# kscalelabs/kbot-joystick

Measured on NVIDIA B200. Metric: env-steps/sec (obs + LSTM actor/critic + torque + terminations + rewards + GAE), higher is better.
Workload: dtype f32 (tcgen05 2xFP16-split GEMMs, fp32 accumulate)

## Files before the change

### kbot-joystick_b200/csrc/kbs_api.cu

```cuda
#include <math.h>
#include <stdio.h>
#include <stdlib.h>
#include <string.h>

#include <new>

#include "kbs_common.cuh"

namespace {

inline int64_t round_up4(int64_t n) { return (n + 3) / 4 * 4; }

int check_ld(int64_t ld, int64_t n) {
  if (n <= 0) return KBS_E_SHAPE;
  if (ld < round_up4(n)) return KBS_E_SHAPE;
  if (ld % 4) return KBS_E_ALIGN;
  return KBS_OK;
}

#define REQ(p)            \
  do {                    \
    if (!(p)) return KBS_E_NULL; \
  } while (0)
#define AL(p)                                     \
  do {                                            \
    if ((p) && !kbs_aligned16(p)) return KBS_E_ALIGN; \
  } while (0)

int check_state(const kbs_state_view* s, int64_t n, bool need_priv) {
  REQ(s);
  REQ(s->qpos); REQ(s->qvel);
  int rc = check_ld(s->ld, n);
  if (rc) return rc;
  AL(s->qpos); AL(s->qvel); AL(s->sensordata); AL(s->xpos); AL(s->xquat); AL(s->cinert); AL(s->cvel);
  AL(s->actuator_force); AL(s->com_distance); AL(s->time);
  if (need_priv) { REQ(s->sensordata); REQ(s->xpos); REQ(s->xquat); }
  return KBS_OK;
}

kbs_state_view state_at(const kbs_state_view& s, int64_t t) {
  kbs_state_view o = s;
  const int64_t ld = s.ld;
  if (s.qpos) o.qpos = s.qpos + t * KBS_NQ * ld;
  if (s.qvel) o.qvel = s.qvel + t * KBS_NV * ld;
  if (s.sensordata) o.sensordata = s.sensordata + t * KBS_NSENSORDATA * ld;
  if (s.xpos) o.xpos = s.xpos + t * 3 * KBS_NBODY * ld;
  if (s.xquat) o.xquat = s.xquat + t * 4 * KBS_NBODY * ld;
  if (s.cinert) o.cinert = s.cinert + t * 10 * KBS_NBODY * ld;
  if (s.cvel) o.cvel = s.cvel + t * 6 * KBS_NBODY * ld;
  if (s.actuator_force) o.actuator_force = s.actuator_force + t * KBS_NUM_JOINTS * ld;
  if (s.com_distance) o.com_distance = s.com_distance + t * ld;
  if (s.time) o.time = s.time + t * ld;
  return o;
}

kbs_noise_view noise_at(const kbs_noise_view& z, int64_t t, int64_t ld) {
  kbs_noise_view o = z;
  if (z.eps_jpos) o.eps_jpos = z.eps_jpos + t * 20 * ld;
  if (z.eps_jvel) o.eps_jvel = z.eps_jvel + t * 20 * ld;
  if (z.eps_gyro) o.eps_gyro = z.eps_gyro + t * 3 * ld;
  if (z.eps_pg) o.eps_pg = z.eps_pg + t * 3 * ld;
  return o;
}

size_t trunk_scratch_floats(const kbs_handle* h, int64_t n) {
  return h->p.gemm_path != KBS_GEMM_SIMT_FP32 ? kbs_tc_scratch_floats(h, n) : kbs_simt_scratch_floats(h, n);
}

int trunk(kbs_handle* h, int net, const float* obs, int64_t ld, float* carry, const uint8_t* done, float* out_rm,
          int64_t n, cudaStream_t st) {
  if (h->p.gemm_path == KBS_GEMM_SIMT_FP32) return kbs_simt_trunk(h, net, obs, ld, carry, done, out_rm, n, st);
  const size_t H = size_t(h->p.hidden_size);
  float* ws = h->scratch;
  float* x_rm = ws + kbs_tc_scratch_floats(h, n) - 2 * size_t(n) * H - 256;
  float* hbuf = x_rm + size_t(n) * H;
  int rc;
  if ((rc = kbs_simt_in_proj(h, net, obs, ld, x_rm, n, st))) return rc;
  if ((rc = kbs_tc_lstm_stack(h, net, x_rm, carry, done, hbuf, ws, n, false, st))) return rc;
  return kbs_simt_out_proj(h, net, hbuf, out_rm, n, st);
}

constexpr int kOutLd = 64;

int rollout_fused_tc(kbs_handle* h, const kbs_rollout_io* io, int64_t n, cudaStream_t st) {
  const int64_t ld = io->state.ld, T = io->T;
  const bool critic = io->value != nullptr;
  int chunks_cfg = 1;
  {
    const char* e = getenv("KBS_ROLLOUT_CHUNKS");
    chunks_cfg = e ? atoi(e) : 1;
    if (chunks_cfg < 1 || chunks_cfg > kKbsMaxChunks) chunks_cfg = 1;
  }
  const int64_t CT = (T + chunks_cfg - 1) / chunks_cfg;
  const size_t sbf = size_t(kbs_tc_sb_floats(h, n));
  const size_t ws_f = kbs_tc_rollout_ws_floats(h, n);
  const size_t lag_f = io->pg_carry ? size_t(T) * 3 * ld : 0;
  const size_t aobs_f = io->actor_obs ? 0 : size_t(T) * KBS_ACTOR_OBS * ld;
  const size_t cobs_f = critic ? size_t(CT) * KBS_CRITIC_OBS * ld : 0;
  const size_t xsb_f = size_t(T) * sbf;
  const size_t osb_a_f = size_t(kbs_tc_obs_sb_floats(h, KBS_NET_ACTOR, n, CT));
  const size_t osb_c_f = critic ? size_t(kbs_tc_obs_sb_floats(h, KBS_NET_CRITIC, n, CT)) : 0;
  int rc = kbs_scratch_reserve(h, ws_f + lag_f + aobs_f + cobs_f + xsb_f * (critic ? 2 : 1) + osb_a_f + osb_c_f + 64);
  if (rc) return rc;
  float* ws = h->scratch;
  float* lagged = io->pg_carry ? ws + ws_f : nullptr;
  float* aobs = io->actor_obs ? io->actor_obs : ws + ws_f + lag_f;
  float* cobs = critic ? ws + ws_f + lag_f + aobs_f : nullptr;
  float* xsb_a = ws + ws_f + lag_f + aobs_f + cobs_f;
  float* xsb_c = critic ? xsb_a + xsb_f : nullptr;
  float* osb_a = xsb_a + xsb_f * (critic ? 2 : 1);
  float* osb_c = critic ? osb_a + osb_a_f : nullptr;

  if ((rc = kbs_launch_terminate(h, io->state, io->term_codes, io->done, io->success, nullptr, n, st, T))) return rc;
  if (lagged) {
    if ((rc = kbs_launch_phase_a_scans(h, io->command, io->u_switch, io->cmd_mode, io->cmd_u6, io->cmd_u_arms, io->done,
                                       io->state.sensordata, io->episode.pg_lag, io->pg_carry, lagged, T, ld, n, st)))
      return rc;
  } else if ((rc = kbs_launch_command_scan(h, io->command, io->u_switch, io->cmd_mode, io->cmd_u6, io->cmd_u_arms, io->done,
                                           T, ld, n, st))) {
    return rc;
  }
  if ((rc = kbs_side_stream_init(h))) return rc;
  const bool overlap = chunks_cfg > 1;
  cudaStream_t aux = overlap ? h->aux_stream : st;
  if (overlap) {
    KBS_CUDA_TRY(cudaEventRecord(h->ev_pre, st));
    KBS_CUDA_TRY(cudaStreamWaitEvent(aux, h->ev_pre, 0));
  }
  KbsTcRolloutArgs r{};
  r.x_sb_all[0] = xsb_a; r.x_sb_all[1] = xsb_c;
  int n_chunks = 0;
  for (int64_t t0 = 0; t0 < T; t0 += CT, ++n_chunks) {
    const int64_t tc = (T - t0 < CT) ? T - t0 : CT;
    const kbs_state_view s = state_at(io->state, t0);
    const kbs_noise_view nz = noise_at(io->noise, t0, ld);
    float* aobs_c = aobs + t0 * KBS_ACTOR_OBS * ld;
    if ((rc = kbs_launch_observations(h, s, &nz, &io->episode, io->command + t0 * KBS_NUM_COMMANDS * ld, nullptr, nullptr,
                                      nullptr, aobs_c, cobs, n, aux, tc, lagged ? lagged + t0 * 3 * ld : nullptr,
                                      true)))
      return rc;
    const float* obs_soa[2] = {aobs_c, cobs};
    float* obs_sb[2] = {osb_a, osb_c};
    float* xsb[2] = {xsb_a + size_t(t0) * sbf, critic ? xsb_c + size_t(t0) * sbf : nullptr};
    if ((rc = kbs_tc_input_proj_all(h, critic ? 2 : 1, obs_soa, obs_sb, xsb, ld, n, tc, aux,
                                    critic ? s.cinert : nullptr, critic ? s.cvel : nullptr, chunks_cfg == 1 ? &r : nullptr)))
      return rc;
    if (overlap) KBS_CUDA_TRY(cudaEventRecord(h->ev_chunk[n_chunks], aux));
  }

  r.chunk_len = overlap ? CT : 0; r.chunk_events = h->ev_chunk;
  r.n = n; r.ld = ld; r.T = T; r.with_critic = critic;
  r.carry[0] = io->actor_carry; r.carry[1] = io->critic_carry;
  r.done = io->done; r.actor_obs = aobs; r.lpf = io->lpf; r.eps_action = io->eps_action;
  r.qpos = io->state.qpos; r.qvel = io->state.qvel; r.ep = io->episode;
  r.action = io->action; r.log_prob = io->log_prob; r.ctrl = io->ctrl; r.value = io->value;
  r.ws = ws;
  return kbs_tc_rollout_recurrent(h, r, st);
}

}

int kbs_side_stream_init(kbs_handle* h) {
  if (h->side_stream) return 0;
  KBS_CUDA_TRY(cudaStreamCreateWithFlags(&h->side_stream, cudaStreamNonBlocking));
  KBS_CUDA_TRY(cudaStreamCreateWithFlags(&h->aux_stream, cudaStreamNonBlocking));
  KBS_CUDA_TRY(cudaEventCreateWithFlags(&h->ev_pre, cudaEventDisableTiming));
  for (int i = 0; i < kKbsMaxChunks; ++i) KBS_CUDA_TRY(cudaEventCreateWithFlags(&h->ev_chunk[i], cudaEventDisableTiming));
  for (int i = 0; i < 2; ++i) {
    KBS_CUDA_TRY(cudaEventCreateWithFlags(&h->ev_lstm[i], cudaEventDisableTiming));
    KBS_CUDA_TRY(cudaEventCreateWithFlags(&h->ev_head[i], cudaEventDisableTiming));
  }
  return 0;
}

int kbs_status_init(kbs_handle* h) {
  if (h->persist_status) return KBS_OK;
  KBS_CUDA_TRY(cudaMalloc(&h->persist_status, 256));
  KBS_CUDA_TRY(cudaMemset(h->persist_status, 0, 256));
  KBS_CUDA_TRY(cudaHostAlloc(&h->status_host, 64, cudaHostAllocDefault));
  *h->status_host = 0u;
  return KBS_OK;
}

int kbs_status_publish(kbs_handle* h, cudaStream_t st) {
  if (!h->persist_status) return KBS_OK;
  KBS_CUDA_TRY(cudaMemcpyAsync(h->status_host, h->persist_status, 4, cudaMemcpyDeviceToHost, st));
  return KBS_OK;
}

int kbs_enter(kbs_handle* h) {
  int dev = -1;
  KBS_CUDA_TRY(cudaGetDevice(&dev));
  if (dev != h->device) return KBS_E_STATE;
  if (h->status_host && *reinterpret_cast<volatile unsigned int*>(h->status_host) != 0u) return KBS_E_DEVICE;
  return KBS_OK;
}

int kbs_scratch_reserve(kbs_handle* h, size_t floats) {
  if (floats <= h->scratch_floats) return KBS_OK;
  if (h->scratch_locked) return KBS_E_STATE;
  if (h->scratch) { KBS_CUDA_TRY(cudaFree(h->scratch)); h->scratch = nullptr; h->scratch_floats = 0; }
  const size_t want = floats + floats / 8 + 1024;
  KBS_CUDA_TRY(cudaMalloc(&h->scratch, want * sizeof(float)));
  h->scratch_floats = want;
  return KBS_OK;
}

extern "C" {

int kbs_version(void) { return KBS_VERSION; }

const char* kbs_error_string(int code) {
  switch (code) {
    case KBS_OK: return "ok";
    case KBS_E_NULL: return "required pointer is NULL";
    case KBS_E_SHAPE: return "unsupported shape (n_envs / ld / T / hidden_size)";
    case KBS_E_ALIGN: return "pointer not 16-byte aligned or ld % 4 != 0";
    case KBS_E_STATE: return "handle not ready (weights not packed, or datapath unavailable)";
    case KBS_E_PARAM: return "bad scalar parameter";
    case KBS_E_DEVICE: return "device health word set (dependency-wait timeout or FP16-split operand out of range): kbs_device_status";
    default: return code > 0 ? cudaGetErrorString((cudaError_t)code) : "unknown kbs error";
  }
}

int kbs_default_params(kbs_params* p) {
  REQ(p);
  memset(p, 0, sizeof(*p));
  p->hidden_size = 256; p->depth = 2; p->gemm_path = KBS_GEMM_SIMT_FP32; p->normalize_advantages = 0;
  p->ctrl_dt = 0.02f; p->min_std = 0.01f; p->max_std = 1.0f; p->var_scale = 0.5f;
  {
    const double w = 2.0 * M_PI * 10.0, dt = 0.02;
    p->lpf_alpha = (float)(w * dt / (1.0 + w * dt));
  }
  p->gamma = 0.94f; p->lam = 0.94f; p->adv_eps = 1e-6f;
  p->jpos_noise_mag = (float)(3.0 * M_PI / 180.0); p->jvel_noise_mag = (float)(15.0 * M_PI / 180.0);
  p->gyro_noise_std = (float)(10.0 * M_PI / 180.0); p->pg_noise_std = (float)(3.0 * M_PI / 180.0);
// ... 337 lines not shown
  return kbs_launch_torque(h, action, *s, ep, ctrl_out, n, (cudaStream_t)stream);
}

int kbs_torque_substeps(kbs_handle* h, const float* action, float* prev_action, const float* u_drop, const float* latency,
                        const float* q_sub, const float* qd_sub, const kbs_episode_view* ep, float* ctrl_out, int32_t n_substeps,
                        float sub_dt, float drop_prob, int64_t ld, int64_t n, void* stream) {
  REQ(h); REQ(action); REQ(prev_action); REQ(u_drop); REQ(latency); REQ(q_sub); REQ(qd_sub); REQ(ctrl_out);
  if (n_substeps <= 0 || n_substeps > 64) return KBS_E_SHAPE;
  int rc = check_ld(ld, n);
  if (rc) return rc;
  AL(action); AL(prev_action); AL(u_drop); AL(latency); AL(q_sub); AL(qd_sub); AL(ctrl_out);
  return kbs_launch_torque_substeps(h, action, prev_action, u_drop, latency, q_sub, qd_sub, ep, ctrl_out, n_substeps, sub_dt,
                                    drop_prob, ld, n, (cudaStream_t)stream);
}

int kbs_terminate(kbs_handle* h, const kbs_state_view* s, int32_t* codes, uint8_t* done, uint8_t* success, float* pre,
                  int64_t n, void* stream) {
  REQ(h);
  int rc = check_state(s, n, false);
  if (rc) return rc;
  REQ(s->xpos); REQ(s->time);
  AL(codes); AL(pre);
  if ((reinterpret_cast<uintptr_t>(done) & 3u) || (reinterpret_cast<uintptr_t>(success) & 3u)) return KBS_E_ALIGN;
  return kbs_launch_terminate(h, *s, codes, done, success, pre, n, (cudaStream_t)stream);
}

int kbs_rewards(kbs_handle* h, const kbs_traj_view* traj, const kbs_reward_carry* carry, float* total,
                float* components, int64_t n, void* stream) {
  REQ(h); REQ(traj); REQ(carry); REQ(total);
  if (traj->T <= 0 || traj->T > 65535) return KBS_E_SHAPE;
  int rc = check_state(&traj->state, n, true);
  if (rc) return rc;
  REQ(traj->state.com_distance); REQ(traj->command); REQ(traj->ctrl); REQ(traj->done);
  REQ(carry->t_single); REQ(carry->airtime); REQ(carry->prev_contact);
  AL(traj->command); AL(traj->ctrl); AL(total); AL(components);
  if (reinterpret_cast<uintptr_t>(traj->done) & 3u) return KBS_E_ALIGN;
  return kbs_launch_rewards(h, *traj, *carry, total, components, n, (cudaStream_t)stream);
}

int kbs_gae(kbs_handle* h, const float* values, const float* rewards, const uint8_t* done, const uint8_t* success,
            float* advantages, float* value_targets, int64_t T, int64_t ld, int64_t n, void* stream) {
  REQ(h); REQ(values); REQ(rewards); REQ(done); REQ(success); REQ(advantages); REQ(value_targets);
  if (T <= 0) return KBS_E_SHAPE;
  if (n <= 0 || ld < n) return KBS_E_SHAPE;
  return kbs_launch_gae(h, values, rewards, done, success, advantages, value_targets, T, ld, n, (cudaStream_t)stream);
}

int kbs_policy_step(kbs_handle* h, const float* joint_angles, const float* joint_vel, const float* projected_gravity,
                    const float* gyro, const float* command, const float* carry_in, float* carry_out,
                    float* action_out, int64_t n, void* stream) {
  REQ(h); REQ(joint_angles); REQ(joint_vel); REQ(projected_gravity); REQ(gyro); REQ(command); REQ(carry_in);
  REQ(carry_out); REQ(action_out);
  if (n <= 0) return KBS_E_SHAPE;
  { const int rc0 = kbs_enter(h); if (rc0) return rc0; }
  cudaStream_t st = (cudaStream_t)stream;
  const int H = h->p.hidden_size, d2 = 2 * h->p.depth;
  const int64_t ld = round_up4(n);
  {
    const char* legacy_env = getenv("KBS_TC_PER_STEP");
    if (h->p.gemm_path != KBS_GEMM_SIMT_FP32 && !(legacy_env && atoi(legacy_env)) && d2 <= 8 &&
        kbs_tc_persistent_available(h, n, 1, 1)) {
      const int carry_w = d2 * H + 20;
      const size_t ws_f = kbs_tc_rollout_ws_floats(h, n);
      const size_t xsb_f = size_t(kbs_tc_sb_floats(h, n));
      const size_t osb_f = size_t(kbs_tc_obs_sb_floats(h, KBS_NET_ACTOR, n, 1));
      int rc = kbs_scratch_reserve(h, ws_f + xsb_f + osb_f + size_t(KBS_ACTOR_OBS + 20 + 20) * ld + 64);
      if (rc) return rc;
      float* ws = h->scratch;
      float* xsb = ws + ws_f;
      float* osb = xsb + xsb_f;
      float* obs = osb + osb_f;
      float* lpf = obs + size_t(KBS_ACTOR_OBS) * ld;
      float* act = lpf + 20 * ld;
      if ((rc = kbs_launch_policy_pack(h, joint_angles, joint_vel, projected_gravity, gyro, command, carry_in, obs, nullptr,
                                       lpf, ld, n, st)))
        return rc;
      const float* obs_soa[2] = {obs, nullptr};
      float* obs_sb[2] = {osb, nullptr};
      float* x_all[2] = {xsb, nullptr};
      KbsTcRolloutArgs r{};
      if ((rc = kbs_tc_input_proj_all(h, 1, obs_soa, obs_sb, x_all, ld, n, 1, st, nullptr, nullptr, &r))) return rc;
      r.n = n; r.ld = ld; r.T = 1; r.with_critic = false;
      r.carry[0] = const_cast<float*>(carry_in); r.carry_out[0] = carry_out; r.carry_ld = carry_w;
      r.actor_obs = obs; r.lpf = lpf; r.action = act;
      r.ws = ws;
      if ((rc = kbs_tc_rollout_recurrent(h, r, st))) return rc;
      return kbs_launch_policy_unpack(h, nullptr, lpf, act, carry_out, action_out, ld, n, st);
    }
  }
  const size_t ts = trunk_scratch_floats(h, n);
  const size_t need = ts + size_t(n) * kOutLd + size_t(KBS_ACTOR_OBS + 20 + 20) * ld + size_t(d2) * n * H + 64;
  int rc = kbs_scratch_reserve(h, need);
  if (rc) return rc;
  float* out_rm = h->scratch + ts;
  float* obs = out_rm + size_t(n) * kOutLd;
  float* lpf = obs + size_t(KBS_ACTOR_OBS) * ld;
  float* mean = lpf + 20 * ld;
  float* carry = mean + 20 * ld;
  if ((rc = kbs_launch_policy_pack(h, joint_angles, joint_vel, projected_gravity, gyro, command, carry_in, obs, carry,
                                   lpf, ld, n, st)))
    return rc;
  if ((rc = trunk(h, KBS_NET_ACTOR, obs, ld, carry, nullptr, out_rm, n, st))) return rc;
  kbs_actor_out o{};
  o.mean = mean;
  if ((rc = kbs_launch_actor_head(h, out_rm, kOutLd, obs, ld, lpf, nullptr, nullptr, nullptr, o, n, st))) return rc;
  return kbs_launch_policy_unpack(h, carry, lpf, mean, carry_out, action_out, ld, n, st);
}

static int ppo_variables_pass(kbs_handle* h, const kbs_ppo_io* io, int64_t n, cudaStream_t st, size_t base, size_t* end_out,
                              bool dry) {
  int rc;
  const bool critic = io->critic_obs != nullptr;
  const int64_t ld = io->ld, T = io->T;
  if (h->p.gemm_path == KBS_GEMM_SIMT_FP32) {
    const size_t ts = trunk_scratch_floats(h, n);
    if (end_out) *end_out = ts + size_t(n) * kOutLd;
    if (dry) return KBS_OK;
    float* out_rm = h->scratch + ts;
    for (int64_t t = 0; t < T; ++t) {
      const uint8_t* done_t = io->done + t * ld;
      if ((rc = trunk(h, KBS_NET_ACTOR, io->actor_obs + t * KBS_ACTOR_OBS * ld, ld, io->actor_carry, done_t, out_rm, n, st)))
        return rc;
      kbs_actor_out o{};
      o.log_prob = io->log_probs ? io->log_probs + t * ld : nullptr;
      o.entropy = io->entropy ? io->entropy + t * ld : nullptr;
      o.std = io->action_std ? io->action_std + t * KBS_NUM_JOINTS * ld : nullptr;
      o.mean = io->mean ? io->mean + t * KBS_NUM_JOINTS * ld : nullptr;
      if ((rc = kbs_launch_actor_head(h, out_rm, kOutLd, io->actor_obs + t * KBS_ACTOR_OBS * ld, ld, io->lpf, nullptr,
                                      io->action + t * KBS_NUM_JOINTS * ld, done_t, o, n, st)))
        return rc;
      if (critic) {
        if ((rc = trunk(h, KBS_NET_CRITIC, io->critic_obs + t * KBS_CRITIC_OBS * ld, ld, io->critic_carry, done_t, out_rm,
                        n, st)))
          return rc;
        if ((rc = kbs_launch_critic_head(h, out_rm, kOutLd, io->values + t * ld, n, st))) return rc;
      }
    }
    return KBS_OK;
  }
  const size_t sbf = size_t(kbs_tc_sb_floats(h, n));
  const size_t ws_f = kbs_tc_rollout_ws_floats(h, n), xsb_f = size_t(T) * sbf;
  const size_t osb_a_f = size_t(kbs_tc_obs_sb_floats(h, KBS_NET_ACTOR, n, T));
  const size_t osb_c_f = critic ? size_t(kbs_tc_obs_sb_floats(h, KBS_NET_CRITIC, n, T)) : 0;
  if (end_out) *end_out = base + ws_f + xsb_f * (critic ? 2 : 1) + osb_a_f + osb_c_f + 64;
  if (dry) return KBS_OK;
  float* ws = h->scratch + base;
  float* xsb_a = ws + ws_f;
  float* xsb_c = critic ? xsb_a + xsb_f : nullptr;
  float* osb_a = xsb_a + xsb_f * (critic ? 2 : 1);
  float* osb_c = critic ? osb_a + osb_a_f : nullptr;
  KbsTcRolloutArgs r{};
  {
    const float* obs_soa[2] = {io->actor_obs, io->critic_obs};
    float* obs_sb[2] = {osb_a, osb_c};
    float* xsb[2] = {xsb_a, xsb_c};
    if ((rc = kbs_tc_input_proj_all(h, critic ? 2 : 1, obs_soa, obs_sb, xsb, ld, n, T, st, nullptr, nullptr, &r))) return rc;
  }
  r.n = n; r.ld = ld; r.T = T; r.with_critic = critic;
  r.carry[0] = io->actor_carry; r.carry[1] = io->critic_carry;
  r.done = io->done; r.actor_obs = io->actor_obs; r.lpf = io->lpf;
  r.action_in = io->action; r.log_prob = io->log_probs; r.entropy = io->entropy; r.action_std = io->action_std;
  r.mean = io->mean;
  r.value = io->values;
  r.ws = ws;
  return kbs_tc_rollout_recurrent(h, r, st);
}

int kbs_ppo_variables(kbs_handle* h, const kbs_ppo_io* io, int64_t n, void* stream) {
  REQ(h); REQ(io);
  REQ(io->actor_obs); REQ(io->action); REQ(io->done); REQ(io->actor_carry); REQ(io->lpf); REQ(io->log_probs);
  REQ(io->entropy);
  if (io->T <= 0) return KBS_E_SHAPE;
  int rc = check_ld(io->ld, n);
  if (rc) return rc;
  if ((rc = kbs_enter(h))) return rc;
  const bool critic = io->critic_obs != nullptr;
  if (critic) { REQ(io->critic_carry); REQ(io->values); }
  AL(io->actor_obs); AL(io->critic_obs); AL(io->action); AL(io->lpf); AL(io->log_probs); AL(io->values); AL(io->entropy);
  AL(io->action_std); AL(io->mean);
  const bool mirror = io->actor_obs_mirror != nullptr;
  if (mirror) {
    REQ(io->actor_mirror_carry); REQ(io->lpf_mirror); REQ(io->action_mirror_loss);
    if (io->critic_obs_mirror) { REQ(io->critic_mirror_carry); REQ(io->value_mirror_loss); if (!critic) return KBS_E_NULL; }
    AL(io->actor_obs_mirror); AL(io->critic_obs_mirror); AL(io->lpf_mirror); AL(io->action_mirror_loss); AL(io->value_mirror_loss);
  }
  cudaStream_t st = (cudaStream_t)stream;
  const int64_t ld = io->ld, T = io->T;
  const bool tc = h->p.gemm_path != KBS_GEMM_SIMT_FP32;
  if (tc && io->mean && !kbs_tc_persistent_available(h, n, T, critic ? 2 : 1)) return KBS_E_SHAPE;
  const size_t mir_f = mirror ? (2 * size_t(T) * KBS_NUM_JOINTS * ld + 3 * size_t(T) * ld + 255) / 256 * 256 : 0;
  size_t pass_end = 0;
  if ((rc = ppo_variables_pass(h, io, n, st, tc ? mir_f : 0, &pass_end, true))) return rc;
  if ((rc = kbs_scratch_reserve(h, pass_end + (tc ? 0 : mir_f) + 64))) return rc;
  float* mir = mirror ? (tc ? h->scratch : h->scratch + pass_end) : nullptr;
  kbs_ppo_io a = *io;
  if (mirror && !a.mean) a.mean = mir;
  if ((rc = ppo_variables_pass(h, &a, n, st, tc ? mir_f : 0, nullptr, false))) return rc;
  if (!mirror) return KBS_OK;
  float* mean_m = mir + size_t(T) * KBS_NUM_JOINTS * ld;
  float* value_m = mean_m + size_t(T) * KBS_NUM_JOINTS * ld;
  float* lp_m = value_m + size_t(T) * ld;
  float* ent_m = lp_m + size_t(T) * ld;
  kbs_ppo_io m = *io;
  m.actor_obs = io->actor_obs_mirror; m.critic_obs = io->critic_obs_mirror;
  m.actor_carry = io->actor_mirror_carry; m.critic_carry = io->critic_mirror_carry; m.lpf = io->lpf_mirror;
  m.log_probs = lp_m; m.entropy = ent_m; m.values = io->critic_obs_mirror ? value_m : nullptr; m.action_std = nullptr;
  m.mean = mean_m;
  if ((rc = ppo_variables_pass(h, &m, n, st, tc ? mir_f : 0, nullptr, false))) return rc;
  return kbs_launch_mirror_loss(h, a.mean, mean_m, io->values, value_m, io->action_mirror_loss,
                                io->critic_obs_mirror ? io->value_mirror_loss : nullptr, io->actor_mirror_loss_scale,
                                io->critic_mirror_loss_scale, T, ld, n, st);
}

int kbs_generate_rollout_noise(kbs_handle* h, uint64_t seed, int64_t step0, const kbs_noise_view* noise, float* eps_action,
                               float* u_switch, int32_t* cmd_mode, float* cmd_u6, float* cmd_u_arms, int64_t T, int64_t ld, int64_t n,
                               void* stream) {
  REQ(h);
  if (T <= 0 || T > 65535) return KBS_E_SHAPE;
  int rc = check_ld(ld, n);
  if (rc) return rc;
  if (noise) { AL(noise->eps_jpos); AL(noise->eps_jvel); AL(noise->eps_gyro); AL(noise->eps_pg); }
  AL(eps_action); AL(u_switch); AL(cmd_mode); AL(cmd_u6); AL(cmd_u_arms);
  return kbs_launch_rollout_noise(h, seed, step0, noise, eps_action, u_switch, cmd_mode, cmd_u6, cmd_u_arms, T, ld, n,
                                  (cudaStream_t)stream);
}

int kbs_adamw_default_params(kbs_adamw_params* p) {
  REQ(p);
  p->lr = 5e-4f; p->b1 = 0.9; p->b2 = 0.999; p->eps = 1e-8f;
  p->weight_decay = 1e-5f;
  p->grad_scale = 1.0f;
  p->max_grad_norm = 10.0f;
  return KBS_OK;
}

int kbs_actuator_rand_default_params(kbs_actuator_rand_params* p) {
  REQ(p);
  p->kp_scale = 1.4f; p->kd_scale = 1.4f; p->torque_limit_scale_low = 0.5f; p->action_bias_scale = 0.02f;
  p->torque_bias_scale = 0.0f;
  return KBS_OK;
}

int kbs_sample_actuator_randomization(kbs_handle* h, const kbs_actuator_rand_params* rp, const float* u, const uint8_t* reset,
// ... 65 lines not shown
```

### kbot-joystick_b200/csrc/kbs_common.cuh

```cuda
#pragma once
#include <cuda_runtime.h>
#include <stdint.h>

#include "kbotstep.h"

#if defined(__CUDA_ARCH__) && (__CUDA_ARCH__ < 1000)
#error "libkbotstep is written for sm_100a (B200) only"
#endif

#define KBS_CUDA_TRY(expr)                      \
  do {                                          \
    cudaError_t _e = (expr);                    \
    if (_e != cudaSuccess) return (int)_e;      \
  } while (0)

#define KBS_LAUNCH_CHECK()                      \
  do {                                          \
    cudaError_t _e = cudaPeekAtLastError();     \
    if (_e != cudaSuccess) return (int)_e;      \
  } while (0)

struct KbsNet {
  bool packed = false;
  int num_in = 0, num_out = 0;
  int kin_pad = 0;
  int nout_pad = 0;
  float* w_in = nullptr;
  float* b_in = nullptr;
  float* w_ih[KBS_MAX_DEPTH] = {nullptr, nullptr, nullptr, nullptr};
  float* w_hh[KBS_MAX_DEPTH] = {nullptr, nullptr, nullptr, nullptr};
  float* b[KBS_MAX_DEPTH] = {nullptr, nullptr, nullptr, nullptr};
  float* w_out = nullptr;
  float* b_out = nullptr;
  float* tc_image = nullptr;
  size_t tc_image_floats = 0;
  float* tc_bwd_image = nullptr;
  float* tc_bwd_image64 = nullptr;
  float* tc_fwd8_image = nullptr;
};

enum KbsKernelId {
  KBS_K_OBS = 0, KBS_K_COMMAND, KBS_K_TORQUE, KBS_K_TERMINATE, KBS_K_REWARD_ROT, KBS_K_REWARD_TERMS, KBS_K_REWARD_SCAN,
  KBS_K_GAE, KBS_K_ADV_NORM, KBS_K_POLICY_IO, KBS_K_GEMM_SIMT, KBS_K_LSTM_CELL, KBS_K_ACTOR_HEAD, KBS_K_CRITIC_HEAD,
  KBS_K_PACK, KBS_K_LSTM_TC, KBS_K_PROJ_TC, KBS_K_ROLLOUT_TC, KBS_K_BPTT_TC, KBS_K_GEMM_TN, KBS_K_PACK_TN, KBS_K_TN_REDUCE, KBS_K_COUNT
};
constexpr int kKbsProfMaxPairs = 8192;
constexpr int kKbsMaxChunks = 8;

struct kbs_handle {
  kbs_params p;
  int device = 0;
  int num_sms = 148;
  KbsNet net[2];
  float* scratch = nullptr;
  size_t scratch_floats = 0;
  int64_t launches = 0;
  bool prof_on = false;
  int prof_n = 0;
  cudaEvent_t* prof_ev = nullptr;
  int8_t* prof_id = nullptr;
  cudaStream_t side_stream = nullptr;
  cudaStream_t aux_stream = nullptr;
  cudaEvent_t ev_pre = nullptr, ev_chunk[8] = {};
  cudaEvent_t ev_lstm[2] = {nullptr, nullptr}, ev_head[2] = {nullptr, nullptr};
  double* norm_partial = nullptr;
  unsigned int* loss_ticket = nullptr;
  unsigned int* persist_status = nullptr;
  unsigned int* status_host = nullptr;
  bool tc_attr_set = false;
  bool head_attr_set = false;
  bool bptt_attr_set = false;
  bool fwd_save_attr_set = false;
  bool dw_attr_set = false;
  cudaEvent_t ev_critic_ready = nullptr;
  bool scratch_locked = false;
  long long* trace_buf = nullptr;
  int64_t trace_step = -1;
  int trace_layer = 0;
};

struct KbsLaunchScope {
  kbs_handle* h; cudaStream_t st; int slot;
  KbsLaunchScope(kbs_handle* h_, int id, cudaStream_t st_) : h(h_), st(st_), slot(-1) {
    h->launches++;
    if (h->prof_on && h->prof_n < kKbsProfMaxPairs) {
      slot = h->prof_n++;
      h->prof_id[slot] = (int8_t)id;
      cudaEventRecord(h->prof_ev[2 * slot], st);
    }
  }
  ~KbsLaunchScope() { if (slot >= 0) cudaEventRecord(h->prof_ev[2 * slot + 1], st); }
};
#define KBS_LAUNCH(h, id, st, ...) do { KbsLaunchScope _ls((h), (id), (st)); __VA_ARGS__; } while (0)

int kbs_side_stream_init(kbs_handle* h);
int kbs_status_init(kbs_handle* h);
int kbs_status_publish(kbs_handle* h, cudaStream_t st);
int kbs_enter(kbs_handle* h);
int kbs_scratch_reserve(kbs_handle* h, size_t floats);

int kbs_launch_observations(kbs_handle* h, const kbs_state_view& s, const kbs_noise_view* nz,
                            const kbs_episode_view* ep, const float* command, float* pg_carry,
                            const uint8_t* pg_reset, float* computed, float* actor_obs, float* critic_obs, int64_t n,
                            cudaStream_t st, int64_t T = 1, const float* pg_lagged = nullptr, bool skip_dump = false);
int kbs_launch_ppo_loss(kbs_handle* h, const kbs_ppo_loss_params& L, const kbs_ppo_loss_io& io, int64_t n, cudaStream_t st);
int kbs_launch_ppo_loss_at(kbs_handle* h, const kbs_ppo_loss_params& L, const kbs_ppo_loss_io& io, int64_t n, double* partials,
                           cudaStream_t st);
int kbs_launch_com_distance(kbs_handle* h, const int32_t* geom1, const int32_t* geom2, const float* pos, const float* com,
                            float* out, int ncon, int64_t T, int64_t ld, int64_t n, cudaStream_t st);
int kbs_launch_mirror_obs(kbs_handle* h, const kbs_state_view& s, const float* computed, const float* command,
                          float* actor_obs, float* critic_obs, float* command_out, int64_t n, int64_t T, cudaStream_t st);
int kbs_launch_mirror_joints(kbs_handle* h, const float* in, float* out, int64_t ld, int64_t n, int64_t T, cudaStream_t st);
int kbs_launch_command(kbs_handle* h, const float* cmd_in, float* cmd_out, const float* u_switch,
                       const int32_t* mode, const float* u6, const float* u_arms, const uint8_t* done, int64_t ld,
                       int64_t n, cudaStream_t st);
int kbs_launch_command_scan(kbs_handle* h, float* command, const float* u_switch, const int32_t* mode, const float* u6,
                            const float* u_arms, const uint8_t* done, int64_t T, int64_t ld, int64_t n, cudaStream_t st);
int kbs_launch_phase_a_scans(kbs_handle* h, float* command, const float* u_switch, const int32_t* mode, const float* u6,
                             const float* u_arms, const uint8_t* done, const float* sensordata, const float* lag,
                             float* pg_carry, float* lagged, int64_t T, int64_t ld, int64_t n, cudaStream_t st);
int kbs_launch_pg_scan(kbs_handle* h, const float* sensordata, const float* lag, const uint8_t* done, float* pg_carry,
                       float* lagged, int64_t T, int64_t ld, int64_t n, cudaStream_t st);
int kbs_launch_torque(kbs_handle* h, const float* action, const kbs_state_view& s, const kbs_episode_view* ep,
                      float* ctrl, int64_t n, cudaStream_t st);
int kbs_launch_torque_substeps(kbs_handle* h, const float* action, float* prev_action, const float* u_drop, const float* latency,
                               const float* q_sub, const float* qd_sub, const kbs_episode_view* ep, float* ctrl, int S, float sub_dt,
                               float drop_prob, int64_t ld, int64_t n, cudaStream_t st);
int kbs_launch_mirror_loss(kbs_handle* h, const float* mean, const float* mean_m, const float* value, const float* value_m,
                           float* action_loss, float* value_loss, float scale_a, float scale_c, int64_t T, int64_t ld, int64_t n,
                           cudaStream_t st);
int kbs_launch_actuator_rand(kbs_handle* h, const kbs_actuator_rand_params& rp, const float* u, const uint8_t* reset,
                             const kbs_episode_view& ep, int64_t ld, int64_t n, cudaStream_t st);
int kbs_launch_rollout_noise(kbs_handle* h, uint64_t seed, int64_t step0, const kbs_noise_view* nz, float* eps_action, float* u_switch,
                             int32_t* cmd_mode, float* cmd_u6, float* cmd_u_arms, int64_t T, int64_t ld, int64_t n, cudaStream_t st);
int kbs_launch_terminate(kbs_handle* h, const kbs_state_view& s, int32_t* codes, uint8_t* done, uint8_t* success,
                         float* pre, int64_t n, cudaStream_t st, int64_t T = 1);
int kbs_launch_rewards(kbs_handle* h, const kbs_traj_view& tr, const kbs_reward_carry& carry, float* total,
                       float* components, int64_t n, cudaStream_t st);
int kbs_launch_gae(kbs_handle* h, const float* values, const float* rewards, const uint8_t* done,
                   const uint8_t* success, float* adv, float* targets, int64_t T, int64_t ld, int64_t n,
                   cudaStream_t st);
int kbs_launch_policy_pack(kbs_handle* h, const float* ja, const float* jv, const float* pg, const float* gyro,
                           const float* cmd, const float* carry_in, float* obs_soa, float* carry_aos, float* lpf_soa,
                           int64_t ld, int64_t n, cudaStream_t st);
int kbs_launch_policy_unpack(kbs_handle* h, const float* carry_aos, const float* lpf_soa, const float* mean_soa,
                             float* carry_out, float* action_out, int64_t ld, int64_t n, cudaStream_t st);

int kbs_simt_pack(kbs_handle* h, int net, const kbs_net_weights* w, cudaStream_t st);
int kbs_simt_trunk(kbs_handle* h, int net, const float* obs_soa, int64_t ld, float* carry, const uint8_t* done,
                   float* out_rowmajor , int64_t n, cudaStream_t st);
size_t kbs_simt_scratch_floats(const kbs_handle* h, int64_t n);

int kbs_simt_gemm_nt(kbs_handle* h, const float* A, int64_t lda, const float* W, int ldw, const float* bias, float* C, int ldc,
                     int64_t M, int Npad, int K, int accumulate, cudaStream_t st, int batch = 1, int64_t a_ts = 0, int64_t c_ts = 0);
int kbs_simt_gemm_tn(kbs_handle* h, const float* A, int lda, const float* B, int ldb, float* C, int ldc, int M, int N, int64_t K,
                     float* partials, int splits, cudaStream_t st);
int kbs_simt_in_proj(kbs_handle* h, int net, const float* obs_soa, int64_t ld, float* x_rm, int64_t n, cudaStream_t st);
int kbs_simt_out_proj(kbs_handle* h, int net, const float* h_rm, float* out_rm, int64_t n, cudaStream_t st);

int kbs_tc_pack(kbs_handle* h, int net, cudaStream_t st);
size_t kbs_tc_scratch_floats(const kbs_handle* h, int64_t n);
int kbs_tc_lstm_stack(kbs_handle* h, int net, const float* x_rm, float* carry, const uint8_t* done, float* out_h_rm,
                      float* ws, int64_t n, bool carry_sb_valid, cudaStream_t st);
struct KbsTcRolloutArgs {
  int64_t n, ld, T;
  bool with_critic;
  const float* x_sb_all[2];
  bool x_is_obs[2];
  float* carry[2];
  int64_t carry_ld;
  float* carry_out[2];
  const uint8_t* done;
  const float* actor_obs;
  float* lpf;
  const float* eps_action;
  const float* qpos;
  const float* qvel;
  kbs_episode_view ep;
  float* action; float* log_prob; float* ctrl; float* value;
  const float* action_in;
  float* entropy;
  float* action_std;
  float* mean;
  int save;
  char* xmid_hist[2]; char* hsb_hist[2]; float* c_hist[2]; float* save_g[2]; float* sraw;
  float* ws;
  int64_t chunk_len;
  cudaEvent_t* chunk_events;
};
size_t kbs_tc_rollout_ws_floats(const kbs_handle* h, int64_t n);
int64_t kbs_tc_sb_floats(const kbs_handle* h, int64_t n);
int64_t kbs_tc_obs_sb_floats(const kbs_handle* h, int net, int64_t n, int64_t T);
int kbs_tc_input_proj_all(kbs_handle* h, int nets, const float* const* obs_soa, float* const* obs_sb, float* const* x_sb_all,
                          int64_t ld, int64_t n, int64_t T, cudaStream_t st, const float* cinert = nullptr,
                          const float* cvel = nullptr, struct KbsTcRolloutArgs* r_out = nullptr);
bool kbs_tc_fused_input(const kbs_handle* h, int net, int64_t n, int64_t T, int nets);
int kbs_tc_rollout_recurrent(kbs_handle* h, const KbsTcRolloutArgs& r, cudaStream_t st);
bool kbs_tc_persistent_available(const kbs_handle* h, int64_t n, int64_t T, int nets);
int kbs_tc_debug_trace(kbs_handle* h, long long* trace_out, float* ws, int64_t n, cudaStream_t st);
int kbs_tc_gates_fwd(kbs_handle* h, int net, int layer, const void* x_sb, const void* h_sb, float* gates_out, int64_t n,
                     cudaStream_t st);
int kbs_tc_pack_bwd(kbs_handle* h, int net, cudaStream_t st, int tile = 128);
int kbs_tc_bptt_tile(const kbs_handle* h, int64_t n);
int kbs_tc_bwd_gemm(kbs_handle* h, int net, int layer, const void* dG_sb, float* out, int64_t n, float out_scale, cudaStream_t st);
size_t kbs_tc_rows_sb_bytes(const kbs_handle* h, int64_t n, int K);
struct KbsTnPlan { int kb_split, ksplit, kb_total; size_t col_bytes; };
KbsTnPlan kbs_tc_tn_plan(const kbs_handle* h, int64_t rows);
int kbs_tc_pack_tn(kbs_handle* h, const KbsTnPlan& plan, bool b_operand, const float* src, int64_t ld, int col0, int ncols,
                   int ncols_pad, int64_t rows, char* dst, float scale, int ones_col, cudaStream_t st, int64_t n_step = 0,
                   int64_t np_step = 0);
int kbs_tc_gemm_tn(kbs_handle* h, const KbsTnPlan& plan, const char* a_t, int m_panels, int m_valid, const char* b_t, int n_tiles,
                   const char* ones_blk, const float* zero_bias, float* partial, float out_scale, cudaStream_t st);
int kbs_tc_ones_block(kbs_handle* h, char* blk, cudaStream_t st);
int kbs_tc_sb_to_tn(kbs_handle* h, const KbsTnPlan& plan, bool b_operand, const char* src, size_t step_bytes, int kb_src, int blk0,
                    int nblk, int64_t n, int64_t T, char* dst, cudaStream_t st);
int kbs_tc_soa_to_tn(kbs_handle* h, const KbsTnPlan& plan, const float* soa, int F, int64_t ld, int64_t n, int64_t T, int ncols_pad,
                     bool ones, char* dst, cudaStream_t st);
bool kbs_tc_dw_direct_available(const kbs_handle* h, int64_t n);
int kbs_tc_dw_direct(kbs_handle* h, const KbsTnPlan& plan, const char* dG, const char* x_hist, const char* h_hist, int64_t n, int64_t T,
                     float* partial, float out_scale, cudaStream_t st);
struct KbsBpttNet {
  char* dG; const float* save_g; const float* c_hist; const float* dh_top; float* dx; char* dx0; float* dc; unsigned int* flags;
  char* tn_dG[KBS_MAX_DEPTH];
  const float* dv; const float* w_out;
};
struct KbsBpttArgs {
  KbsBpttNet net[2]; int nets; int64_t n, ld, T; const uint8_t* done; float gscale;
  const KbsTnPlan* tn_plan;
  bool* transposed_out;
};
struct KbsFwdSaveNet {
  const char* x0; char* xmid; char* hsb; float* c_hist; float* save_g; float* h_top_rm; unsigned int* flags;
  const float* carry0;
  char* tn_xh[KBS_MAX_DEPTH];
};
struct KbsFwdSaveArgs {
  KbsFwdSaveNet net[2]; int nets; int64_t n, ld, T; const uint8_t* done;
  const KbsTnPlan* tn_plan; bool* transposed_out;
};
size_t kbs_tc_fwd_save_flag_bytes(const kbs_handle* h, int64_t n);
bool kbs_tc_fwd_save_available(const kbs_handle* h, int64_t n, int64_t T);
int kbs_tc_fwd_save(kbs_handle* h, const KbsFwdSaveArgs& f, cudaStream_t st);
size_t kbs_tc_bptt_flag_bytes(const kbs_handle* h, int64_t n);
bool kbs_tc_bptt_available(const kbs_handle* h, int64_t n, int64_t T);
int kbs_tc_bptt(kbs_handle* h, const KbsBpttArgs& a, cudaStream_t st);
int kbs_tc_tn_reduce(kbs_handle* h, const KbsTnPlan& plan, const float* partial, int m_panels, int ldc, int col0, int nrows,
                     int ncols, float* dst, int ld_dst, cudaStream_t st);
int kbs_tc_tn_reduce_multi(kbs_handle* h, const KbsTnPlan& plan, const float* partial, int m_panels, int ldc, int nrows, int nseg,
                           const int (*seg)[3], float* const* dst, cudaStream_t st);
int kbs_tc_kind_of(const kbs_handle* h);
int kbs_tc_debug_gates(kbs_handle* h, int net, int layer, const float* x_rm, const float* h_rm, float* gates_out,
                       float* ws, int64_t n, cudaStream_t st);

int kbs_launch_actor_head(kbs_handle* h, const float* out_rm, int ldo, const float* obs_soa, int64_t ld, float* lpf,
                          const float* eps, const float* action_in, const uint8_t* done, const kbs_actor_out& o,
                          int64_t n, cudaStream_t st);
int kbs_launch_critic_head(kbs_handle* h, const float* out_rm, int ldo, float* value, int64_t n, cudaStream_t st);

__device__ __forceinline__ void kbs_ld4(const float* __restrict__ base, int64_t row, int64_t ld, int64_t n0,
                                        float (&v)[4]) {
  const float4 t = __ldcs(reinterpret_cast<const float4*>(base + row * ld + n0));
  v[0] = t.x; v[1] = t.y; v[2] = t.z; v[3] = t.w;
}
__device__ __forceinline__ void kbs_st4(float* __restrict__ base, int64_t row, int64_t ld, int64_t n0,
                                        const float (&v)[4]) {
  __stcs(reinterpret_cast<float4*>(base + row * ld + n0), make_float4(v[0], v[1], v[2], v[3]));
}
__device__ __forceinline__ void kbs_copy4(const float* __restrict__ src, int64_t srow, float* __restrict__ dst,
                                          int64_t drow, int64_t ld, int64_t n0) {
  __stcs(reinterpret_cast<float4*>(dst + drow * ld + n0),
         __ldcs(reinterpret_cast<const float4*>(src + srow * ld + n0)));
}

constexpr int kKbsPanelRows = 128;
enum { KBS_KIND_TF32 = 0, KBS_KIND_F16 = 1 };
constexpr float kKbsF16LoScale = 2048.0f;
inline __host__ __device__ constexpr int kbs_chunk_elems(int kind) { return kind == KBS_KIND_TF32 ? 4 : 8; }
inline __host__ __device__ constexpr int kbs_block_k(int kind) { return 4 * kbs_chunk_elems(kind); }
inline size_t kbs_sb_bytes(int64_t rows_padded, int K) { return size_t(rows_padded) * size_t(K) * 2 * 4; }
// ... 94 lines not shown
```

### kbot-joystick_b200/csrc/kbs_elementwise.cu

```cuda
#include <math.h>

#include "kbs_common.cuh"

namespace {

constexpr int kThreads = 128;
constexpr float kHalfPi = 1.57079632679489662f;
constexpr float kPi = 3.14159265358979324f;

__device__ __forceinline__ void quat_norm_eps(float (&q)[4], float eps) {
  const float n = sqrtf(((q[0] * q[0] + q[1] * q[1]) + q[2] * q[2]) + q[3] * q[3]) + eps;
  q[0] /= n; q[1] /= n; q[2] /= n; q[3] /= n;
}

__device__ __forceinline__ void quat_to_euler(const float (&qin)[4], float eps, float (&e)[3]) {
  float q[4] = {qin[0], qin[1], qin[2], qin[3]};
  quat_norm_eps(q, eps);
  const float w = q[0], x = q[1], y = q[2], z = q[3];
  e[0] = atan2f(2.0f * (w * x + y * z), 1.0f - 2.0f * (x * x + y * y));
  const float sinp = 2.0f * (w * y - z * x);
  e[1] = (fabsf(sinp) >= 1.0f) ? copysignf(kHalfPi, sinp) : asinf(sinp);
  e[2] = atan2f(2.0f * (w * z + x * y), 1.0f - 2.0f * (y * y + z * z));
}

__device__ __forceinline__ void euler_to_quat(float roll, float pitch, float yaw, float (&q)[4]) {
  const float r = roll * 0.5f, p = pitch * 0.5f, y = yaw * 0.5f;
  const float cr = cosf(r), sr = sinf(r), cp = cosf(p), sp = sinf(p), cy = cosf(y), sy = sinf(y);
  q[0] = cr * cp * cy + sr * sp * sy;
  q[1] = sr * cp * cy - cr * sp * sy;
  q[2] = cr * sp * cy + sr * cp * sy;
  q[3] = cr * cp * sy - sr * sp * cy;
  const float n = sqrtf(((q[0] * q[0] + q[1] * q[1]) + q[2] * q[2]) + q[3] * q[3]);
  q[0] /= n; q[1] /= n; q[2] /= n; q[3] /= n;
}

__device__ __forceinline__ void rotate_vec(const float (&v)[3], const float (&qin)[4], bool inverse, float eps,
                                           float (&o)[3]) {
  float q[4] = {qin[0], qin[1], qin[2], qin[3]};
  quat_norm_eps(q, eps);
  const float w = q[0];
  const float x = inverse ? -q[1] : q[1], y = inverse ? -q[2] : q[2], z = inverse ? -q[3] : q[3];
  const float vx = v[0], vy = v[1], vz = v[2];
  const float t = 2.0f;
  o[0] = w * w * vx + t * y * w * vz - t * z * w * vy + x * x * vx + t * y * x * vy + t * z * x * vz - z * z * vx - y * y * vx;
  o[1] = t * x * y * vx + y * y * vy + t * z * y * vz + t * w * z * vx - z * z * vy + w * w * vy - t * w * x * vz - x * x * vy;
  o[2] = t * x * z * vx + t * y * z * vy + z * z * vz - t * w * y * vx + w * w * vz + t * w * x * vy - y * y * vz - x * x * vz;
}

__device__ __forceinline__ bool zero_cmd(float c0, float c1, float c2) {
  return sqrtf((c0 * c0 + c1 * c1) + c2 * c2) < 1e-3f;
}

__device__ __forceinline__ void encode_pg(const float (&g)[3], float (&o)[5]) {
  o[0] = atan2f(g[1], -g[2]);
  o[1] = atan2f(-g[0], sqrtf(g[1] * g[1] + g[2] * g[2]));
  const float n = sqrtf((g[0] * g[0] + g[1] * g[1]) + g[2] * g[2]);
  o[2] = g[0] / n; o[3] = g[1] / n; o[4] = g[2] / n;
}

constexpr int kCopyRowsPerSection = 46;
constexpr int kObsSections = 4;

__global__ void __launch_bounds__(kThreads)
obs_kernel(const __grid_constant__ kbs_params P, kbs_state_view s, kbs_noise_view nz,
           const kbs_episode_view ep, const float* __restrict__ command, float* __restrict__ pg_carry,
           const uint8_t* __restrict__ pg_reset, const float* __restrict__ pg_lagged, float* __restrict__ computed,
           float* __restrict__ actor_obs, float* __restrict__ critic_obs, int64_t n) {
  const int64_t n0 = (int64_t(blockIdx.x) * kThreads + threadIdx.x) * 4;
  if (n0 >= n) return;
  const int64_t ld = s.ld;
  {
    const int64_t t = blockIdx.z;
    s.qpos += t * KBS_NQ * ld; s.qvel += t * KBS_NV * ld; s.sensordata += t * KBS_NSENSORDATA * ld;
    s.xpos += t * 3 * KBS_NBODY * ld; s.xquat += t * 4 * KBS_NBODY * ld;
    if (s.cinert) s.cinert += t * 10 * KBS_NBODY * ld;
    if (s.cvel) s.cvel += t * 6 * KBS_NBODY * ld;
    if (s.actuator_force) s.actuator_force += t * KBS_NUM_JOINTS * ld;
    if (nz.eps_jpos) { nz.eps_jpos += t * 20 * ld; nz.eps_jvel += t * 20 * ld; nz.eps_gyro += t * 3 * ld; nz.eps_pg += t * 3 * ld; }
    command += t * KBS_NUM_COMMANDS * ld;
    if (pg_lagged) pg_lagged += t * 3 * ld;
    if (computed) computed += t * KBS_NUM_COMPUTED_OBS * ld;
    if (actor_obs) actor_obs += t * KBS_ACTOR_OBS * ld;
    if (critic_obs) critic_obs += t * KBS_CRITIC_OBS * ld;
  }

  const int sec = blockIdx.y;
  if (sec >= kObsSections) {
    const int i0 = (sec - kObsSections) * kCopyRowsPerSection;
#pragma unroll 8
    for (int i = i0; i < i0 + kCopyRowsPerSection; ++i) {
      if (i < 230) kbs_copy4(s.cinert, 10 + i, critic_obs, 80 + i, ld, n0);
      else if (i < 368) kbs_copy4(s.cvel, 6 + (i - 230), critic_obs, 310 + (i - 230), ld, n0);
    }
    return;
  }

  const bool has_noise = nz.eps_jpos != nullptr;

  if (sec < 2) {
#pragma unroll 5
  for (int j = sec * 10; j < sec * 10 + 10; ++j) {
    float q[4], qd[4], jb[4] = {0, 0, 0, 0}, e1[4] = {0, 0, 0, 0}, e2[4] = {0, 0, 0, 0};
    kbs_ld4(s.qpos, 7 + j, ld, n0, q);
    kbs_ld4(s.qvel, 6 + j, ld, n0, qd);
    if (ep.jpos_bias) kbs_ld4(ep.jpos_bias, j, ld, n0, jb);
    if (has_noise) { kbs_ld4(nz.eps_jpos, j, ld, n0, e1); kbs_ld4(nz.eps_jvel, j, ld, n0, e2); }
    float bj[4], nbj[4], nv[4], a0[4], a1[4], c0[4], c1[4];
#pragma unroll
    for (int l = 0; l < 4; ++l) {
      bj[l] = q[l] + jb[l];
      nbj[l] = bj[l] + P.jpos_noise_mag * e1[l];
      nv[l] = qd[l] + P.jvel_noise_mag * e2[l];
      a0[l] = (nbj[l] - P.joint_bias[j]) / P.joint_range[j];
      a1[l] = nv[l] / 10.0f;
      c0[l] = (q[l] - P.joint_bias[j]) / P.joint_range[j];
      c1[l] = qd[l] / 10.0f;
    }
    if (computed) { kbs_st4(computed, j, ld, n0, bj); kbs_st4(computed, 20 + j, ld, n0, nbj); kbs_st4(computed, 40 + j, ld, n0, nv); }
    if (actor_obs) { kbs_st4(actor_obs, j, ld, n0, a0); kbs_st4(actor_obs, 20 + j, ld, n0, a1); }
    if (critic_obs) { kbs_st4(critic_obs, j, ld, n0, c0); kbs_st4(critic_obs, 20 + j, ld, n0, c1); }
  }
  return;
  }

  if (sec == 2) {
    float iq[4][4], gy[3][4];
#pragma unroll
    for (int k = 0; k < 4; ++k) kbs_ld4(s.sensordata, P.sd_imu_quat + k, ld, n0, iq[k]);
#pragma unroll
    for (int k = 0; k < 3; ++k) kbs_ld4(s.sensordata, P.sd_gyro + k, ld, n0, gy[k]);
    float lag[4] = {0, 0, 0, 0}, pgb[3][4] = {}, epg[3][4] = {}, egy[3][4] = {}, prev[3][4];
    if (ep.pg_lag) kbs_ld4(ep.pg_lag, 0, ld, n0, lag);
    if (ep.pg_bias) { for (int k = 0; k < 3; ++k) kbs_ld4(ep.pg_bias, k, ld, n0, pgb[k]); }
    if (has_noise) {
      for (int k = 0; k < 3; ++k) { kbs_ld4(nz.eps_pg, k, ld, n0, epg[k]); kbs_ld4(nz.eps_gyro, k, ld, n0, egy[k]); }
    }
    if (pg_carry) { for (int k = 0; k < 3; ++k) kbs_ld4(pg_carry, k, ld, n0, prev[k]); }
    float lagged[3][4];
    if (pg_lagged) { for (int k = 0; k < 3; ++k) kbs_ld4(pg_lagged, k, ld, n0, lagged[k]); }
    bool rs[4] = {false, false, false, false};
    if (pg_reset) {
      const uchar4 r4 = *reinterpret_cast<const uchar4*>(pg_reset + n0);
      rs[0] = r4.x != 0; rs[1] = r4.y != 0; rs[2] = r4.z != 0; rs[3] = r4.w != 0;
    }
    float o_pg[3][4], o_ipg[3][4], o_nipg[3][4], o_ngy[3][4], o_carry[3][4], enc_a[5][4], enc_c[5][4];
#pragma unroll
    for (int l = 0; l < 4; ++l) {
      const float q[4] = {iq[0][l], iq[1][l], iq[2][l], iq[3][l]};
      const float g[3] = {0.0f, 0.0f, -P.gravity};
      float gb[3];
      rotate_vec(g, q, true, P.eps_quat, gb);
      float na[3];
#pragma unroll
      for (int k = 0; k < 3; ++k) {
        const float pv = (pg_carry && !rs[l]) ? prev[k][l] : gb[k];
        const float nc = pg_lagged ? lagged[k][l] : lag[l] * pv + (1.0f - lag[l]) * gb[k];
        o_carry[k][l] = nc;
        o_pg[k][l] = gb[k];
        o_ipg[k][l] = nc + pgb[k][l];
        o_nipg[k][l] = o_ipg[k][l] + P.pg_noise_std * epg[k][l];
        o_ngy[k][l] = gy[k][l] + P.gyro_noise_std * egy[k][l];
        na[k] = o_nipg[k][l];
      }
      float ea[5], ec[5];
      encode_pg(na, ea);
      encode_pg(gb, ec);
#pragma unroll
      for (int k = 0; k < 5; ++k) { enc_a[k][l] = ea[k]; enc_c[k][l] = ec[k]; }
    }
    if (pg_carry) { for (int k = 0; k < 3; ++k) kbs_st4(pg_carry, k, ld, n0, o_carry[k]); }
    if (computed) {
      for (int k = 0; k < 3; ++k) {
        kbs_st4(computed, 60 + k, ld, n0, o_ngy[k]);
        kbs_st4(computed, 69 + k, ld, n0, o_pg[k]);
        kbs_st4(computed, 72 + k, ld, n0, o_ipg[k]);
        kbs_st4(computed, 75 + k, ld, n0, o_nipg[k]);
      }
    }
    if (actor_obs) {
      for (int k = 0; k < 5; ++k) kbs_st4(actor_obs, 40 + k, ld, n0, enc_a[k]);
      for (int k = 0; k < 3; ++k) kbs_st4(actor_obs, 45 + k, ld, n0, o_ngy[k]);
    }
    if (critic_obs) {
      for (int k = 0; k < 5; ++k) kbs_st4(critic_obs, 40 + k, ld, n0, enc_c[k]);
      for (int k = 0; k < 3; ++k) kbs_st4(critic_obs, 45 + k, ld, n0, gy[k]);
    }
  }

  if (sec == 2) {
  float c[16][4];
#pragma unroll
  for (int k = 0; k < 16; ++k) kbs_ld4(command, k, ld, n0, c[k]);
  float zc[4];
#pragma unroll
  for (int l = 0; l < 4; ++l) zc[l] = zero_cmd(c[0][l], c[1][l], c[2][l]) ? 1.0f : 0.0f;
  if (actor_obs) {
    kbs_st4(actor_obs, 48, ld, n0, zc);
#pragma unroll
    for (int k = 0; k < 16; ++k) kbs_st4(actor_obs, 49 + k, ld, n0, c[k]);
  }
  if (critic_obs) {
    kbs_st4(critic_obs, 48, ld, n0, zc);
#pragma unroll
    for (int k = 0; k < 16; ++k) kbs_st4(critic_obs, 49 + k, ld, n0, c[k]);
  }
  return;
  }

  if (computed || critic_obs) {
    float bp[3][4], lp[3][4], rp[3][4], bq[4][4], fpos[6][4];
#pragma unroll
    for (int k = 0; k < 3; ++k) {
      kbs_ld4(s.xpos, 3 * P.body_base + k, ld, n0, bp[k]);
      kbs_ld4(s.xpos, 3 * P.body_lfoot + k, ld, n0, lp[k]);
      kbs_ld4(s.xpos, 3 * P.body_rfoot + k, ld, n0, rp[k]);
    }
#pragma unroll
    for (int k = 0; k < 4; ++k) kbs_ld4(s.xquat, 4 * P.body_base + k, ld, n0, bq[k]);
#pragma unroll
    for (int l = 0; l < 4; ++l) {
      const float q[4] = {bq[0][l], bq[1][l], bq[2][l], bq[3][l]};
      float e[3], qy[4], o[3];
      quat_to_euler(q, P.eps_quat, e);
      euler_to_quat(0.0f, 0.0f, e[2], qy);
      const float dl[3] = {lp[0][l] - bp[0][l], lp[1][l] - bp[1][l], lp[2][l] - bp[2][l]};
      rotate_vec(dl, qy, true, P.eps_quat, o);
      fpos[0][l] = o[0]; fpos[1][l] = o[1]; fpos[2][l] = o[2];
      const float dr[3] = {rp[0][l] - bp[0][l], rp[1][l] - bp[1][l], rp[2][l] - bp[2][l]};
      rotate_vec(dr, qy, true, P.eps_quat, o);
      fpos[3][l] = o[0]; fpos[4][l] = o[1]; fpos[5][l] = o[2];
    }
    if (computed) { for (int k = 0; k < 6; ++k) kbs_st4(computed, 63 + k, ld, n0, fpos[k]); }
    if (critic_obs) {
      for (int k = 0; k < 6; ++k) kbs_st4(critic_obs, 67 + k, ld, n0, fpos[k]);
      kbs_copy4(s.sensordata, P.sd_touch_l, critic_obs, 65, ld, n0);
      kbs_copy4(s.sensordata, P.sd_touch_r, critic_obs, 66, ld, n0);
      for (int k = 0; k < 7; ++k) kbs_copy4(s.qpos, k, critic_obs, 73 + k, ld, n0);
      for (int k = 0; k < 6; ++k) kbs_copy4(s.qvel, k, critic_obs, 448 + k, ld, n0);
#pragma unroll 4
      for (int j = 0; j < KBS_NUM_JOINTS; ++j) {
        float f[4];
        kbs_ld4(s.actuator_force, j, ld, n0, f);
#pragma unroll
        for (int l = 0; l < 4; ++l) f[l] = f[l] / 4.0f;
        kbs_st4(critic_obs, 454 + j, ld, n0, f);
      }
      kbs_st4(critic_obs, 474, ld, n0, bp[2]);
    }
  }
}

__device__ __forceinline__ int mirror_src_joint(int j) { return j < 5 ? j + 5 : (j < 10 ? j - 5 : j); }

__global__ void __launch_bounds__(kThreads)
mirror_obs_kernel(const __grid_constant__ kbs_params P, kbs_state_view s, const float* __restrict__ computed,
                  const float* __restrict__ command, float* __restrict__ actor_obs, float* __restrict__ critic_obs,
                  float* __restrict__ command_out, int64_t n) {
  const int64_t n0 = (int64_t(blockIdx.x) * kThreads + threadIdx.x) * 4;
  if (n0 >= n) return;
  const int64_t ld = s.ld;
  {
    const int64_t t = blockIdx.z;
    s.qpos += t * KBS_NQ * ld; s.qvel += t * KBS_NV * ld; s.sensordata += t * KBS_NSENSORDATA * ld;
    s.xpos += t * 3 * KBS_NBODY * ld;
    if (s.cinert) s.cinert += t * 10 * KBS_NBODY * ld;
    if (s.cvel) s.cvel += t * 6 * KBS_NBODY * ld;
    if (s.actuator_force) s.actuator_force += t * KBS_NUM_JOINTS * ld;
    computed += t * KBS_NUM_COMPUTED_OBS * ld;
    command += t * KBS_NUM_COMMANDS * ld;
    if (actor_obs) actor_obs += t * KBS_ACTOR_OBS * ld;
    if (critic_obs) critic_obs += t * KBS_CRITIC_OBS * ld;
    if (command_out) command_out += t * KBS_NUM_COMMANDS * ld;
  }
  if (blockIdx.y > 0) {
    const int i0 = (blockIdx.y - 1) * kCopyRowsPerSection;
    for (int i = i0; i < i0 + kCopyRowsPerSection; ++i) {
      float v[4];
      if (i < 230) {
        const int c = i % 10;
        const float sg = (c == 2 || c == 7 || c == 9) ? -1.0f : 1.0f;
        kbs_ld4(s.cinert, 10 + i, ld, n0, v);
#pragma unroll
        for (int l = 0; l < 4; ++l) v[l] = v[l] * sg;
        kbs_st4(critic_obs, 80 + i, ld, n0, v);
      } else if (i < 368) {
        const int c = (i - 230) % 6;
        const float sg = (c & 1) ? -1.0f : 1.0f;
// ... 912 lines not shown
          const float v = lo + u[i] * (hi - lo);
          bool on;
          if (k == 0) on = (m[i] == 0) || (m[i] == 3);
          else if (k == 1) on = (m[i] == 1) || (m[i] == 3);
          else if (k == 2) on = (m[i] == 2) || (m[i] == 3);
          else on = (m[i] == 4);
          c = on ? v : 0.0f;
        } else {
          const float arm = (lo + u[i] * (hi - lo)) * ((u[i] < 0.5f) ? 1.0f : 0.0f);
          c = (m[i] == 3 || m[i] == 4) ? arm : 0.0f;
        }
      }
      command[((t + 1) * KBS_NUM_COMMANDS + k) * ld + e] = c;
    }
  }
}

__device__ __forceinline__ void
pg_scan_body(const kbs_params& P, const float* __restrict__ sensordata, const float* __restrict__ lag_p,
               const uint8_t* __restrict__ done, float* __restrict__ pg_carry, float* __restrict__ lagged, int64_t T,
               int64_t ld, int64_t n) {
  const int64_t e = int64_t(blockIdx.x) * kThreads + threadIdx.x;
  if (e >= n) return;
  const float lag = lag_p ? lag_p[e] : 0.0f;
  float x[3] = {pg_carry[e], pg_carry[ld + e], pg_carry[2 * ld + e]};
  constexpr int kB = 8;
  for (int64_t t0 = 0; t0 < T; t0 += kB) {
    float qv[kB][4];
    bool rsv[kB];
#pragma unroll
    for (int i = 0; i < kB; ++i) {
      const int64_t t = t0 + i < T ? t0 + i : T - 1;
      const float* sd = sensordata + (t * KBS_NSENSORDATA + P.sd_imu_quat) * ld + e;
      qv[i][0] = sd[0]; qv[i][1] = sd[ld]; qv[i][2] = sd[2 * ld]; qv[i][3] = sd[3 * ld];
      rsv[i] = (t > 0) && (done[(t - 1) * ld + e] != 0);
    }
#pragma unroll
    for (int i = 0; i < kB; ++i) {
      const int64_t t = t0 + i;
      if (t >= T) break;
      const float q[4] = {qv[i][0], qv[i][1], qv[i][2], qv[i][3]};
      const float g[3] = {0.0f, 0.0f, -P.gravity};
      float gb[3];
      rotate_vec(g, q, true, P.eps_quat, gb);
#pragma unroll
      for (int k = 0; k < 3; ++k) {
        const float pv = rsv[i] ? gb[k] : x[k];
        x[k] = lag * pv + (1.0f - lag) * gb[k];
        lagged[(t * 3 + k) * ld + e] = x[k];
      }
    }
  }
  pg_carry[e] = x[0]; pg_carry[ld + e] = x[1]; pg_carry[2 * ld + e] = x[2];
}

__global__ void __launch_bounds__(kThreads)
command_scan_kernel(const __grid_constant__ kbs_params P, float* __restrict__ command, const float* __restrict__ u_switch,
                    const int32_t* __restrict__ mode, const float* __restrict__ u6, const float* __restrict__ u_arms,
                    const uint8_t* __restrict__ done, int64_t T, int64_t ld, int64_t n) {
  command_scan_body(P, blockIdx.y, command, u_switch, mode, u6, u_arms, done, T, ld, n);
}
__global__ void __launch_bounds__(kThreads)
pg_scan_kernel(const __grid_constant__ kbs_params P, const float* __restrict__ sensordata, const float* __restrict__ lag_p,
               const uint8_t* __restrict__ done, float* __restrict__ pg_carry, float* __restrict__ lagged, int64_t T,
               int64_t ld, int64_t n) {
  pg_scan_body(P, sensordata, lag_p, done, pg_carry, lagged, T, ld, n);
}
__global__ void __launch_bounds__(kThreads, 4)
phase_a_scans_kernel(const __grid_constant__ kbs_params P, float* __restrict__ command, const float* __restrict__ u_switch,
                     const int32_t* __restrict__ mode, const float* __restrict__ u6, const float* __restrict__ u_arms,
                     const uint8_t* __restrict__ done, const float* __restrict__ sensordata, const float* __restrict__ lag_p,
                     float* __restrict__ pg_carry, float* __restrict__ lagged, int64_t T, int64_t ld, int64_t n) {
  if (blockIdx.y < KBS_NUM_COMMANDS) command_scan_body(P, blockIdx.y, command, u_switch, mode, u6, u_arms, done, T, ld, n);
  else pg_scan_body(P, sensordata, lag_p, done, pg_carry, lagged, T, ld, n);
}

inline unsigned groups4(int64_t n) { return unsigned((((n + 3) / 4) + kThreads - 1) / kThreads); }

}

int kbs_launch_observations(kbs_handle* h, const kbs_state_view& s, const kbs_noise_view* nz,
                            const kbs_episode_view* ep, const float* command, float* pg_carry,
                            const uint8_t* pg_reset, float* computed, float* actor_obs, float* critic_obs, int64_t n,
                            cudaStream_t st, int64_t T, const float* pg_lagged, bool skip_dump) {
  kbs_noise_view z{};
  kbs_episode_view e{};
  if (nz) z = *nz;
  if (ep) e = *ep;
  dim3 grid(groups4(n), (critic_obs && !skip_dump) ? kObsSections + 368 / kCopyRowsPerSection : kObsSections, unsigned(T));
  KBS_LAUNCH(h, KBS_K_OBS, st, (obs_kernel<<<grid, kThreads, 0, st>>>(h->p, s, z, e, command, pg_carry, pg_reset, pg_lagged,
                                                                      computed, actor_obs, critic_obs, n)));
  KBS_LAUNCH_CHECK();
  return KBS_OK;
}

static int ppo_loss_blocks(const kbs_handle* h, const kbs_ppo_loss_io& io) {
  const int64_t total = io.T * io.ld;
  int blocks = int((total + kLossThreads * 8 - 1) / (kLossThreads * 8));
  if (blocks > 4 * h->num_sms) blocks = 4 * h->num_sms;
  return blocks < 1 ? 1 : blocks;
}

int kbs_launch_ppo_loss(kbs_handle* h, const kbs_ppo_loss_params& L, const kbs_ppo_loss_io& io, int64_t n, cudaStream_t st) {
  const int blocks = ppo_loss_blocks(h, io);
  int rc = kbs_scratch_reserve(h, size_t(blocks) * 8 + 16);
  if (rc) return rc;
  return kbs_launch_ppo_loss_at(h, L, io, n, reinterpret_cast<double*>(h->scratch), st);
}

int kbs_launch_ppo_loss_at(kbs_handle* h, const kbs_ppo_loss_params& L, const kbs_ppo_loss_io& io, int64_t n, double* partials,
                           cudaStream_t st) {
  const int blocks = ppo_loss_blocks(h, io);
  if (!h->loss_ticket) {
    KBS_CUDA_TRY(cudaMalloc(&h->loss_ticket, 256));
    KBS_CUDA_TRY(cudaMemsetAsync(h->loss_ticket, 0, 256, st));
  }
  KBS_LAUNCH(h, KBS_K_GAE, st, (ppo_loss_kernel<<<blocks, kLossThreads, 0, st>>>(L, io, n, partials, h->loss_ticket)));
  KBS_LAUNCH_CHECK();
  return KBS_OK;
}

int kbs_launch_com_distance(kbs_handle* h, const int32_t* geom1, const int32_t* geom2, const float* pos, const float* com,
                            float* out, int ncon, int64_t T, int64_t ld, int64_t n, cudaStream_t st) {
  if (ncon < 3 || ncon > kMaxContacts) return KBS_E_SHAPE;
  dim3 grid(unsigned((n + kThreads - 1) / kThreads), unsigned(T));
  KBS_LAUNCH(h, KBS_K_OBS, st, (com_distance_kernel<<<grid, kThreads, 0, st>>>(geom1, geom2, pos, com, out, ncon, ld, n)));
  KBS_LAUNCH_CHECK();
  return KBS_OK;
}

int kbs_launch_mirror_obs(kbs_handle* h, const kbs_state_view& s, const float* computed, const float* command,
                          float* actor_obs, float* critic_obs, float* command_out, int64_t n, int64_t T, cudaStream_t st) {
  dim3 grid(groups4(n), critic_obs ? 1 + 368 / kCopyRowsPerSection : 1, unsigned(T));
  KBS_LAUNCH(h, KBS_K_OBS, st, (mirror_obs_kernel<<<grid, kThreads, 0, st>>>(h->p, s, computed, command, actor_obs, critic_obs,
                                                                             command_out, n)));
  KBS_LAUNCH_CHECK();
  return KBS_OK;
}

int kbs_launch_mirror_joints(kbs_handle* h, const float* in, float* out, int64_t ld, int64_t n, int64_t T, cudaStream_t st) {
  dim3 grid(groups4(n), KBS_NUM_JOINTS, unsigned(T));
  KBS_LAUNCH(h, KBS_K_OBS, st, (mirror_joints_kernel<<<grid, kThreads, 0, st>>>(in, out, ld, n)));
  KBS_LAUNCH_CHECK();
  return KBS_OK;
}

int kbs_launch_command(kbs_handle* h, const float* cmd_in, float* cmd_out, const float* u_switch,
                       const int32_t* mode, const float* u6, const float* u_arms, const uint8_t* done, int64_t ld,
                       int64_t n, cudaStream_t st) {
  KBS_LAUNCH(h, KBS_K_COMMAND, st, (command_kernel<<<groups4(n), kThreads, 0, st>>>(h->p, cmd_in, cmd_out, u_switch,
                                                                                    mode, u6, u_arms, done, ld, n)));
  KBS_LAUNCH_CHECK();
  return KBS_OK;
}

int kbs_launch_command_scan(kbs_handle* h, float* command, const float* u_switch, const int32_t* mode, const float* u6,
                            const float* u_arms, const uint8_t* done, int64_t T, int64_t ld, int64_t n, cudaStream_t st) {
  KBS_LAUNCH(h, KBS_K_COMMAND, st,
             (command_scan_kernel<<<dim3(unsigned((n + kThreads - 1) / kThreads), KBS_NUM_COMMANDS), kThreads, 0, st>>>(h->p, command, u_switch, mode,
                                                                                              u6, u_arms, done, T, ld, n)));
  KBS_LAUNCH_CHECK();
  return KBS_OK;
}

int kbs_launch_phase_a_scans(kbs_handle* h, float* command, const float* u_switch, const int32_t* mode, const float* u6,
                             const float* u_arms, const uint8_t* done, const float* sensordata, const float* lag,
                             float* pg_carry, float* lagged, int64_t T, int64_t ld, int64_t n, cudaStream_t st) {
  KBS_LAUNCH(h, KBS_K_COMMAND, st,
             (phase_a_scans_kernel<<<dim3(unsigned((n + kThreads - 1) / kThreads), KBS_NUM_COMMANDS + 1), kThreads, 0, st>>>(
                 h->p, command, u_switch, mode, u6, u_arms, done, sensordata, lag, pg_carry, lagged, T, ld, n)));
  KBS_LAUNCH_CHECK();
  return KBS_OK;
}

// ... 135 lines not shown
```

### kbot-joystick_b200/csrc/kbs_net_tc.cu

```cuda
#include <math.h>
#include <cuda.h>
#include <stdlib.h>

#include "kbs_common.cuh"

namespace {

constexpr int kPanelRows = 128;
constexpr int kTileCols = 128;
constexpr int kUnitsPerTile = 32;
#ifndef KBS_STAGES
#define KBS_STAGES 6
#endif
constexpr int kStages = KBS_STAGES;
constexpr int kABlockBytes = 2 * 4 * kPanelRows * 16;
constexpr int kBBlockBytes = 2 * 4 * kTileCols * 16;
constexpr int kStageBytes = kABlockBytes + kBBlockBytes;
static_assert(kABlockBytes == kBBlockBytes, "the two producer lanes copy equal-sized blocks");
constexpr int kIssuers = 3;
constexpr int kProducers = 2;
constexpr int kEpiWarps = 8;
constexpr int kThreadsTC = 32 * (kIssuers + kProducers + kEpiWarps);
constexpr int kMaxBias = 1024;
constexpr int kSmemBytes = kStages * kStageBytes + 2 * kMaxBias * 4 + 256  + 1024 ;
// ... 552 lines not shown
#pragma unroll
    for (int i = 0; i < 10; ++i) out_s[lane * 41 + 10 * g + i] = acc[i] + a.b_out[0][10 * g + i];
  }
  __syncthreads();
  float s_z = 0.0f, s_log = 0.0f;
  constexpr float kHalfLog2Pi = 0.918938533204672742f;
  if (live) {
#pragma unroll
    for (int jj = 0; jj < 5; ++jj) {
      const int j = 5 * g + jj;
      const int64_t o = j * ld + e;
      const float sraw = out_s[lane * 41 + KBS_NUM_JOINTS + j];
      const float sp = fmaxf(sraw, 0.0f) + log1pf(expf(-fabsf(sraw)));
      const float sd = fminf((sp + P.min_std) * P.var_scale, P.max_std);
      float m = out_s[lane * 41 + j] + P.joint_bias[j];
      m = m + in_arm[jj];
      const float y = in_lpf[jj];
      const float yn = y + P.lpf_alpha * (m - y);
      a.lpf[o] = rst ? 0.0f : yn;
      float act = yn;
      if (a.eps) act = yn + sd * in_eps[jj];
      const float a_eval = a.action_in ? in_ain[jj] : act;
      const float z = (a_eval - yn) / sd;
      s_z = s_z + (-0.5f * z * z - kHalfLog2Pi);
      s_log = s_log + logf(sd);
      if (a.action) a.action[o] = act;
      if (a.std) a.std[o] = sd;
      if (!a.ctrl) continue;
      const float target = a.ep.action_bias ? __fadd_rn(act, in_ab[jj]) : act;
      float tau = __fsub_rn(__fmul_rn(in_kp[jj], __fsub_rn(target, in_q[jj])), __fmul_rn(in_kd[jj], in_qd[jj]));
      if (a.ep.torque_bias) tau = __fadd_rn(tau, in_tb[jj]);
      a.ctrl[o] = fminf(fmaxf(tau, -in_lim[jj]), in_lim[jj]);
    }
  }
  part[(g * 32 + lane) * 2] = s_z;
  part[(g * 32 + lane) * 2 + 1] = s_log;
  __syncthreads();
  if (g == 0 && live) {
    float z = 0.0f, l = 0.0f;
#pragma unroll
    for (int w = 0; w < 4; ++w) { z = z + part[(w * 32 + lane) * 2]; l = l + part[(w * 32 + lane) * 2 + 1]; }
    if (a.log_prob) a.log_prob[e] = z - l;
    if (a.entropy) a.entropy[e] = l + float(KBS_NUM_JOINTS) * (0.5f + kHalfLog2Pi);
  }
}

constexpr int kPMaxDepth = 2;
constexpr int kPBiasFloats = 2 * kPMaxDepth * kMaxBias + 2 * 256;
constexpr int kEpiWarpsP = 16;
constexpr int kIssuersP = 1;
constexpr int kProducersP = 1;
constexpr int kThreadsP = 32 * (kIssuersP + kProducersP + kEpiWarpsP + 2);
constexpr int kPHeadPartFloats = 4 * kPanelRows * 2;
constexpr int kTileColsP = 256;
constexpr int kUnitsPerTileP = kTileColsP / 4;
constexpr int kBBlockBytesP = 2 * 4 * kTileColsP * 16;
constexpr int kStageBytesP = kABlockBytes + kBBlockBytesP;
constexpr int kStagesP = 4;
constexpr int kPSmemBytes = kStagesP * kStageBytesP + (kPBiasFloats + kPHeadPartFloats) * 4 + 256  + 1024 ;

struct PNet {
  const char* x_sb_all;
  size_t x0_stride;
  int kb_x0;
  char* hsb;
  char* xmid;
  float* fb;
  const char* w_sb[kPMaxDepth];
  const float* bias_t[kPMaxDepth];
  const char* w_head;
  const float* bias_head;
  unsigned int* flags;
  float* c_hist;
  float* save_g;
};
struct PArgs {
  PNet net[2];
  int nets, depth, H, panels, tiles;
  int gpanels;
  int64_t n, ld, T;
  size_t sbb;
  const uint8_t* done;
  const float* arm_cmd;
  float* lpf;
  const float* eps;
  const float* q; const float* qd;
  kbs_episode_view ep;
  float* action; float* log_prob; float* ctrl; float* value;
  const float* action_in; float* entropy; float* std;
  float* mean;
  float* sraw;
  int hist;
  int dbg;
  unsigned int* status;
  long long* trace;
};

struct PItem { int kind, net, layer, panel, tile; int t; bool valid; };
__device__ __forceinline__ PItem p_decode(const PArgs& a, int g) {
  const int lt = a.depth * a.tiles, per_panel = lt + 1, per_net = a.gpanels * per_panel, C = a.nets * per_net;
  const int per_group = (int(a.T) + a.depth) * C;
  const int grp = g / per_group;
  g -= grp * per_group;
  const int s = g / C;
  int i = g - s * C;
  PItem it;
  it.net = i / per_net; i -= it.net * per_net;
  const int pl = i / per_panel;
  it.panel = grp * a.gpanels + pl;
  const int q = i - pl * per_panel;
  if (q < lt) { it.kind = 0; it.layer = q / a.tiles; it.tile = q - it.layer * a.tiles; it.t = s - it.layer; }
  else { it.kind = 1; it.layer = a.depth; it.tile = 0; it.t = s - a.depth; }
  it.valid = it.t >= 0 && it.t < int(a.T) && it.panel < a.panels;
  return it;
}
__device__ __forceinline__ unsigned int ld_volatile_u32(const unsigned int* p) {
  unsigned int v;
  asm volatile("ld.volatile.global.u32 %0, [%1];" : "=r"(v) : "l"(p) : "memory");
  return v;
}
constexpr unsigned long long kPWaitTimeoutNs = 2000000000ull;
__device__ __forceinline__ long long p_wait_deps(const PArgs& a, const PItem& it, bool& drain) {
  if (drain) return 0;
  const PNet& N = a.net[it.net];
  const unsigned int full_l = unsigned(a.tiles * kEpiWarpsP), full_h = unsigned(kEpiWarpsP);
  const unsigned int* fp[3]; unsigned int tg[3]; int nd = 0;
  const unsigned int t = unsigned(it.t);
  if (it.kind == 0) {
    const int l = it.layer;
    if (t >= 1) { fp[nd] = N.flags + l * a.panels + it.panel; tg[nd++] = t * full_l; }
    if (l >= 1) { fp[nd] = N.flags + (l - 1) * a.panels + it.panel; tg[nd++] = (t + 1) * full_l; }
    if (t >= 2 && !a.hist) {
      fp[nd] = N.flags + (l + 1) * a.panels + it.panel;
      tg[nd++] = (t - 1) * (l + 1 == a.depth ? full_h : full_l);
    }
  } else {
    fp[nd] = N.flags + (a.depth - 1) * a.panels + it.panel; tg[nd++] = (t + 1) * full_l;
    if (t >= 1) { fp[nd] = N.flags + a.depth * a.panels + it.panel; tg[nd++] = t * full_h; }
  }
  if (nd == 0) return 0;
  for (int i = nd; i < 3; ++i) { fp[i] = fp[0]; tg[i] = 0u; }
  const long long c0 = clock64();
  unsigned int polls = 0;
  unsigned long long t0 = 0;
  while (true) {
    const unsigned int v0 = ld_volatile_u32(fp[0]), v1 = ld_volatile_u32(fp[1]), v2 = ld_volatile_u32(fp[2]);
    if (v0 >= tg[0] && v1 >= tg[1] && v2 >= tg[2]) break;
    if ((++polls & 1023u) == 0u) {
      if (ld_volatile_u32(a.status) & 3u) { drain = true; break; }
      unsigned long long now;
      asm volatile("mov.u64 %0, %%globaltimer;" : "=l"(now));
      if (t0 == 0) t0 = now;
      else if (now - t0 > kPWaitTimeoutNs) { atomicOr(a.status, 1u + unsigned(it.kind)); drain = true; break; }
    }
  }
  __threadfence();
  return clock64() - c0;
}

template <int KIND, bool SAVE>
__global__ void __launch_bounds__(kThreadsP, 1)
rollout_persist_kernel(const __grid_constant__ kbs_params P, const __grid_constant__ PArgs args) {
  extern __shared__ uint8_t smem_raw[];
  uint8_t* smem = reinterpret_cast<uint8_t*>((reinterpret_cast<uintptr_t>(smem_raw) + 1023) & ~uintptr_t(1023));
  float* bias_s = reinterpret_cast<float*>(smem + kStagesP * kStageBytesP);
  float* bias_head_s = bias_s + 2 * kPMaxDepth * kMaxBias;
// ... 256 lines not shown
                const int u = hf * 8 + i;
                const float cprev = (&cpre[u >> 2].x)[u & 3];
                ai[i] = sigmoidf_(v[u]); af[i] = sigmoidf_(v[16 + u]); ag[i] = tanhf_(v[32 + u]); ao[i] = sigmoidf_(v[48 + u]);
                cn[i] = af[i] * cprev + ai[i] * ag[i];
                hn[i] = ao[i] * tanhf_(cn[i]);
                if (rst) cn[i] = 0.0f;
              }
#pragma unroll
              for (int i = 0; i < 8; ++i) {
                const int u = hf * 8 + i;
                v[u] = ai[i]; v[16 + u] = af[i]; v[32 + u] = ag[i]; v[48 + u] = ao[i];
              }
            } else {
#pragma unroll
            for (int i = 0; i < 8; ++i) {
              const int u = hf * 8 + i;
              const float cprev = (&cpre[u >> 2].x)[u & 3];
              const float gi_ = v[u], gf = v[16 + u], gg = v[32 + u], go = v[48 + u];
              cn[i] = sigmoidf_(gf) * cprev + sig_mul_tanh(gi_, gg);
              hn[i] = sig_mul_tanh(go, cn[i]);
              if (rst) cn[i] = 0.0f;
            }
            }
            if (!((args.dbg & 4) && hn[0] != 12345.0f)) {
              const int uu = u0 + hf * 8;
              const float h0[4] = {hn[0], hn[1], hn[2], hn[3]}, h1[4] = {hn[4], hn[5], hn[6], hn[7]};
              const KbsSplit4 s0 = sb_split4<KIND>(h0), s1 = sb_split4<KIND>(h1);
              sb_store_split8<kPanelRows, KIND>(x_out, R, uu, kb, s0, s1, false);
              sb_store_split8<kPanelRows, KIND>(h_out, R, uu, kb, s0, s1, rst);
              *reinterpret_cast<float4*>(cdst + fb_offset(R, uu, H)) = make_float4(cn[0], cn[1], cn[2], cn[3]);
              *reinterpret_cast<float4*>(cdst + fb_offset(R, uu + 4, H)) = make_float4(cn[4], cn[5], cn[6], cn[7]);
              if (h_carry) {
                const float z = rst ? 0.0f : 1.0f;
                *reinterpret_cast<float4*>(h_carry + fb_offset(R, uu, H)) = make_float4(z * hn[0], z * hn[1], z * hn[2], z * hn[3]);
                *reinterpret_cast<float4*>(h_carry + fb_offset(R, uu + 4, H)) = make_float4(z * hn[4], z * hn[5], z * hn[6], z * hn[7]);
              }
            }
          }
        }
        if (SAVE) {
          __syncwarp();
          if (lane == 0) asm volatile("red.release.cta.shared::cta.add.u32 [%0], 1;" ::"r"(smem_u32(epi_done)) : "memory");
          published = true;
          if (live && !(args.dbg & 2)) {
            float* sg = N.save_g + (size_t(it.t) * args.depth + it.layer) * 4 * npH;
#pragma unroll
            for (int gate = 0; gate < 4; ++gate)
#pragma unroll
              for (int q = 0; q < 4; ++q)
                *reinterpret_cast<float4*>(sg + gate * npH + fb_offset(R, u0 + 4 * q, H)) =
                    make_float4(v[16 * gate + 4 * q], v[16 * gate + 4 * q + 1], v[16 * gate + 4 * q + 2], v[16 * gate + 4 * q + 3]);
          }
        }
      } else {
        float v[16];
        {
          float cr[16];
          tmem_ld8(tq, v); tmem_ld8(tq + 16, v + 8);
          tmem_ld8(tq + kTileColsP, cr); tmem_ld8(tq + kTileColsP + 16, cr + 8);
          tmem_ld_wait();
#pragma unroll
          for (int i = 0; i < 16; ++i) v[i] += kCorr * cr[i];
        }
        tc_fence_before();
        __syncwarp();
        if (lane == 0) mbar_arrive(&acc_empty[0]);
        const float* bs = bias_head_s + it.net * kTileColsP + colq;
        const int64_t e = R;
        const size_t t = size_t(it.t);
        float s_z = 0.0f, s_log = 0.0f;
        if (it.net == 1) {
          if (live && grp == 0) args.value[t * ld + e] = v[0] + bs[0];
        } else {
          constexpr float kHalfLog2Pi = 0.918938533204672742f;
          if (live) {
            const int j0 = 5 * grp;
            float in_lpf[5], in_eps[5], in_arm[5], in_ain[5], in_q[5], in_qd[5], in_kp[5], in_kd[5], in_lim[5], in_ab[5], in_tb[5];
#pragma unroll
            for (int jj = 0; jj < 5; ++jj) {
              const int jn = j0 + jj;
              const int64_t o = jn * ld + e;
              in_lpf[jj] = __ldcg(args.lpf + o);
              in_eps[jj] = args.eps ? __ldg(args.eps + t * KBS_NUM_JOINTS * ld + o) : 0.0f;
              in_arm[jj] = (jn >= 10) ? __ldg(args.arm_cmd + t * KBS_ACTOR_OBS * ld + (jn - 10) * ld + e) : 0.0f;
              in_ain[jj] = args.action_in ? __ldg(args.action_in + t * KBS_NUM_JOINTS * ld + o) : 0.0f;
              if (args.ctrl) {
                in_q[jj] = __ldg(args.q + t * KBS_NQ * ld + o);
                in_qd[jj] = __ldg(args.qd + t * KBS_NV * ld + o);
                in_kp[jj] = args.ep.kp ? __ldg(args.ep.kp + o) : P.kp[jn];
                in_kd[jj] = args.ep.kd ? __ldg(args.ep.kd + o) : P.kd[jn];
                in_lim[jj] = args.ep.tau_limit ? __ldg(args.ep.tau_limit + o) : P.ctrl_limit[jn];
                in_ab[jj] = args.ep.action_bias ? __ldg(args.ep.action_bias + o) : 0.0f;
                in_tb[jj] = args.ep.torque_bias ? __ldg(args.ep.torque_bias + o) : 0.0f;
              }
            }
#pragma unroll
            for (int jj = 0; jj < 5; ++jj) {
              const int jn = j0 + jj;
              const int64_t o = jn * ld + e;
              const float sraw = v[8 + jj] + bs[16 + jj];
              const float sp = fmaxf(sraw, 0.0f) + log1pf(expf(-fabsf(sraw)));
              const float sd = fminf((sp + P.min_std) * P.var_scale, P.max_std);
              float m = (v[jj] + bs[jj]) + P.joint_bias[jn];
              m = m + in_arm[jj];
              const float y = in_lpf[jj];
              const float yn = y + P.lpf_alpha * (m - y);
              args.lpf[o] = rst ? 0.0f : yn;
              float act = yn;
              if (args.eps) act = yn + sd * in_eps[jj];
              const float a_eval = args.action_in ? in_ain[jj] : act;
              const float z = (a_eval - yn) / sd;
              s_z = s_z + (-0.5f * z * z - kHalfLog2Pi);
              s_log = s_log + logf(sd);
              if (args.action) args.action[t * KBS_NUM_JOINTS * ld + o] = act;
              if (args.std) args.std[t * KBS_NUM_JOINTS * ld + o] = sd;
              if (args.mean) args.mean[t * KBS_NUM_JOINTS * ld + o] = yn;
              if (SAVE && args.sraw) args.sraw[t * KBS_NUM_JOINTS * ld + o] = sraw;
              if (args.ctrl) {
                const float target = args.ep.action_bias ? __fadd_rn(act, in_ab[jj]) : act;
                float tau = __fsub_rn(__fmul_rn(in_kp[jj], __fsub_rn(target, in_q[jj])), __fmul_rn(in_kd[jj], in_qd[jj]));
                if (args.ep.torque_bias) tau = __fadd_rn(tau, in_tb[jj]);
                args.ctrl[t * KBS_NUM_JOINTS * ld + o] = fminf(fmaxf(tau, -in_lim[jj]), in_lim[jj]);
              }
            }
          }
          head_part[(grp * kPanelRows + r) * 2] = s_z;
          head_part[(grp * kPanelRows + r) * 2 + 1] = s_log;
          asm volatile("bar.sync %0, 128;" ::"r"(2 + q4) : "memory");
          if (grp == 0 && live) {
            float z = 0.0f, l = 0.0f;
#pragma unroll
            for (int w = 0; w < 4; ++w) { z = z + head_part[(w * kPanelRows + r) * 2]; l = l + head_part[(w * kPanelRows + r) * 2 + 1]; }
            if (args.log_prob) args.log_prob[t * ld + e] = z - l;
            if (args.entropy) args.entropy[t * ld + e] = l + float(KBS_NUM_JOINTS) * (0.5f + kHalfLog2Pi);
          }
          asm volatile("bar.sync %0, 128;" ::"r"(2 + q4) : "memory");
        }
      }
      const long long ew2 = tr ? clock64() : 0;
      __syncwarp();
      long long ewf = 0;
      if (lane == 0 && !published) {
        asm volatile("red.release.cta.shared::cta.add.u32 [%0], 1;" ::"r"(smem_u32(epi_done)) : "memory");
        if (tr) ewf = clock64();
      }
      if (tr) { const long long ew3 = clock64(); epi_cyc[it.kind] += ew3 - ew1; epi_wait += ew1 - ew0; if (it.kind == 0) { ph[1] += ew2 - ew1; ph[2] += ew3 - ew2; ph[3] += ewf - ew2; } }
      ++j;
    }
    if (tr && threadIdx.x == 32 * (kIssuersP + kProducersP)) { tr[4] = epi_cyc[0]; tr[5] = epi_cyc[1]; tr[6] = epi_wait; tr[8] = ph[0]; tr[9] = ph[1]; tr[10] = ph[2]; tr[11] = ph[3]; }
  }
  tc_fence_before();
  __syncthreads();
  if (tr && threadIdx.x == 0) {
    unsigned long long gt_end;
    asm volatile("mov.u64 %0, %%globaltimer;" : "=l"(gt_end));
    tr[0] = clock64() - t_start;
    tr[15] = (long long)(gt_end - gt_start);
  }
  if (warp == 0) {
    asm volatile("tcgen05.dealloc.cta_group::1.sync.aligned.b32 %0, %1;" ::"r"(tmem_base), "r"(512u));
  }
}

constexpr int kBT = 64;
template <int BT> struct BTile {
  static constexpr int kBBlockBytes = 2 * 4 * BT * 16;
  static constexpr int kStageBytes = kABlockBytes + kBBlockBytes;
// ... 783 lines not shown
  short blk_nvalid[kFMaxBlocks];
  int kb, H;
  int64_t n, n_pad;
  const char* w_sb;
  const float* bias;
  char* x_sb;
  size_t sbb;
  int items;
  unsigned int* status;
  int dbg;
  long long* trace;
};

template <int KIND>
__global__ void __launch_bounds__(kFThreads, 1) input_proj_fused_kernel(const __grid_constant__ FProjArgs a) {
  extern __shared__ uint8_t smem_raw[];
  uint8_t* smem = reinterpret_cast<uint8_t*>((reinterpret_cast<uintptr_t>(smem_raw) + 1023) & ~uintptr_t(1023));
  uint8_t* raw = smem;
  uint8_t* op = smem + kFStagesRaw * kFRawBytes;
  float* bias_s = reinterpret_cast<float*>(op + kFStagesOp * kFOpBytes);
  uint64_t* bars = reinterpret_cast<uint64_t*>(bias_s + 256);
  uint64_t* raw_full = bars;
  uint64_t* raw_empty = raw_full + kFStagesRaw;
  uint64_t* full = raw_empty + kFStagesRaw;
  uint64_t* empty = full + kFStagesOp;
  uint64_t* acc_full = empty + kFStagesOp;
  uint64_t* acc_empty = acc_full + 1;
  uint32_t* tmem_slot = reinterpret_cast<uint32_t*>(acc_empty + 1);

  constexpr int kE = kbs_chunk_elems(KIND), kFeat = 4 * kE;
  constexpr int kBlk = kbs_block_k(KIND);
  const int warp = threadIdx.x >> 5, lane = threadIdx.x & 31;
  const int ppt = int(a.n_pad / kPanelRows);

  if (threadIdx.x == 0) {
    for (int s = 0; s < kFStagesRaw; ++s) { mbar_init(&raw_full[s], 1); mbar_init(&raw_empty[s], kFConvWarps / 2); }
    for (int s = 0; s < kFStagesOp; ++s) { mbar_init(&full[s], 1 + kFConvWarps / 2); mbar_init(&empty[s], 1); }
    mbar_init(acc_full, 1); mbar_init(acc_empty, kFEpiWarps);
    asm volatile("fence.mbarrier_init.release.cluster;" ::: "memory");
  }
  if (warp == 0) {
    asm volatile("tcgen05.alloc.cta_group::1.sync.aligned.shared::cta.b32 [%0], %1;" ::"r"(smem_u32(tmem_slot)), "r"(512u));
    asm volatile("tcgen05.relinquish_alloc_permit.cta_group::1.sync.aligned;");
  }
  tc_fence_before();
  __syncthreads();
  tc_fence_after();
  const uint32_t tmem_base = *tmem_slot;
  long long* tr = a.trace ? a.trace + size_t(148 + blockIdx.x) * 16 : nullptr;
  const long long t_start = clock64();
#define FTR_WAIT(slot, stmt) do { if (tr) { const long long w0_ = clock64(); stmt; tw[slot] += clock64() - w0_; } else { stmt; } } while (0)
  long long tw[2] = {0, 0};

  if (warp == 1) {
    if (lane == 0) {
      uint32_t g = 0;
      for (int item = blockIdx.x; item < a.items; item += gridDim.x) {
        const int t = item / ppt, e0 = (item % ppt) * kPanelRows;
        for (int b = 0; b < a.kb; ++b, ++g) {
          const int sr = g % kFStagesRaw;
          const int src = a.blk_src[b];
          FTR_WAIT(0, mbar_wait(&raw_empty[sr], ((g / kFStagesRaw) & 1) ^ 1));
          mbar_expect_tx(&raw_full[sr], (a.dbg & 4) ? 0u : uint32_t(kFeat * kPanelRows * 4));
          if (!(a.dbg & 4)) {
            const int c1 = t * a.rows_per_step[src] + a.blk_row0[b];
            asm volatile(
                "cp.async.bulk.tensor.2d.shared::cluster.global.mbarrier::complete_tx::bytes [%0], [%1, {%2, %3}], [%4];" ::"r"(
                    smem_u32(raw + size_t(sr) * kFRawBytes)),
                "l"(reinterpret_cast<uint64_t>(&a.tmap[src])), "r"(e0), "r"(c1), "r"(smem_u32(&raw_full[sr]))
                : "memory");
          }
        }
      }
      if (tr) tr[2] = tw[0];
    }
    __syncwarp();
  } else if (warp == 2) {
    if (lane == 0) {
      uint32_t g = 0;
      for (int item = blockIdx.x; item < a.items; item += gridDim.x) {
        for (int b = 0; b < a.kb; ++b, ++g) {
          const int s = g % kFStagesOp;
          FTR_WAIT(0, mbar_wait(&empty[s], ((g / kFStagesOp) & 1) ^ 1));
          mbar_expect_tx(&full[s], uint32_t(kFOpBytes - kABlockBytes));
          bulk_g2s(op + size_t(s) * kFOpBytes + kABlockBytes, a.w_sb + size_t(b) * (kFOpBytes - kABlockBytes),
                   uint32_t(kFOpBytes - kABlockBytes), &full[s]);
        }
      }
      if (tr) tr[3] = tw[0];
    }
    __syncwarp();
  } else if (warp >= kFConvWarp0 && warp < kFConvWarp0 + kFConvWarps) {
    const int cw = warp - kFConvWarp0;
    const int set = cw >> 2;
    const int r = (cw & 3) * 32 + lane;
    uint32_t g = 0;
    bool bad = false;
    for (int item = blockIdx.x; item < a.items; item += gridDim.x) {
      const int64_t e0 = int64_t(item % ppt) * kPanelRows;
      const bool valid = e0 + r < a.n;
      for (int b = 0; b < a.kb; ++b, ++g) {
        if (int(g & 1) != set) continue;
        const int sr = g % kFStagesRaw, s = g % kFStagesOp;
        FTR_WAIT(0, mbar_wait(&raw_full[sr], (g / kFStagesRaw) & 1));
        const float* rf = reinterpret_cast<const float*>(raw + size_t(sr) * kFRawBytes) + r;
        const int nv = int(a.blk_nvalid[b]);
        float x[kFeat];
#pragma unroll
        for (int i = 0; i < kFeat; ++i) x[i] = (valid && i < nv && !(a.dbg & 1)) ? rf[i * kPanelRows] : 0.0f;
        bad = bad || sb_out_of_range<KIND, kFeat>(x);
        __syncwarp();
        if (lane == 0) mbar_arrive(&raw_empty[sr]);
        if (g >= 2) { const uint32_t gp = g - 2; FTR_WAIT(1, mbar_wait(&empty[gp % kFStagesOp], (gp / kFStagesOp) & 1)); }
        uint8_t* sa = op + size_t(s) * kFOpBytes;
        if (!(a.dbg & 1))
#pragma unroll
        for (int c = 0; c < 4; ++c) {
          uint4 hi, lo;
          if (KIND == KBS_KIND_F16) {
            const float x0[4] = {x[(8 * c) % kFeat], x[(8 * c + 1) % kFeat], x[(8 * c + 2) % kFeat], x[(8 * c + 3) % kFeat]};
            const float x1[4] = {x[(8 * c + 4) % kFeat], x[(8 * c + 5) % kFeat], x[(8 * c + 6) % kFeat], x[(8 * c + 7) % kFeat]};
            const KbsSplit4 s0 = sb_split4<KIND>(x0), s1 = sb_split4<KIND>(x1);
            hi = make_uint4(s0.hi.x, s0.hi.y, s1.hi.x, s1.hi.y);
            lo = make_uint4(s0.lo.x, s0.lo.y, s1.lo.x, s1.lo.y);
          } else {
            const float x0[4] = {x[(4 * c) % kFeat], x[(4 * c + 1) % kFeat], x[(4 * c + 2) % kFeat], x[(4 * c + 3) % kFeat]};
            const KbsSplit4 s0 = sb_split4<KIND>(x0);
            hi = s0.hi; lo = s0.lo;
          }
          *reinterpret_cast<uint4*>(sa + c * 2048 + r * 16) = hi;
          *reinterpret_cast<uint4*>(sa + 8192 + c * 2048 + r * 16) = lo;
        }
        asm volatile("fence.proxy.async.shared::cta;" ::: "memory");
        __syncwarp();
        if (lane == 0) mbar_arrive(&full[s]);
      }
    }
    sb_flag_range(a.status, bad);
    if (tr && warp == kFConvWarp0 && lane == 0) { tr[4] = tw[0]; tr[5] = tw[1]; }
  } else if (warp == 0) {
    uint32_t g = 0;
    int j = 0;
    for (int item = blockIdx.x; item < a.items; item += gridDim.x, ++j) {
      FTR_WAIT(1, mbar_wait(acc_empty, (j & 1) ^ 1));
      tc_fence_after();
      const uint32_t d_main = tmem_base, d_corr = tmem_base + 256;
      for (int b = 0; b < a.kb; ++b, ++g) {
        const int s = g % kFStagesOp;
        FTR_WAIT(0, mbar_wait(&full[s], (g / kFStagesOp) & 1));
        tc_fence_after();
        const uint32_t sa = smem_u32(op + size_t(s) * kFOpBytes);
        const uint64_t a_hi = umma_desc(sa, 2048, 128), a_lo = a_hi + (8192 >> 4);
        const uint64_t b_hi = umma_desc(sa + kABlockBytes, 8192, 128), b_lo = b_hi + (4096 >> 4);
        constexpr uint64_t kAStep = 4096 >> 4, kBStep = 16384 >> 4;
        if (elect_one()) {
          const uint32_t acc = b != 0;
          if (!(a.dbg & 2)) {
          umma<KIND, 256>(d_main, a_hi, b_hi, acc);
          umma<KIND, 256>(d_corr, a_lo, b_hi, acc);
          umma<KIND, 256>(d_corr, a_hi, b_lo, 1);
          umma<KIND, 256>(d_main, a_hi + kAStep, b_hi + kBStep, 1);
          umma<KIND, 256>(d_corr, a_lo + kAStep, b_hi + kBStep, 1);
          umma<KIND, 256>(d_corr, a_hi + kAStep, b_lo + kBStep, 1);
          }
          umma_commit(&empty[s]);
        }
        __syncwarp();
      }
      if (elect_one()) umma_commit(acc_full);
      __syncwarp();
    }
    if (tr && lane == 0) { tr[6] = tw[0]; tr[7] = tw[1]; tr[1] = j; }
  } else if (warp >= kFEpiWarp0 && warp < kFEpiWarp0 + kFEpiWarps) {
    const int et = threadIdx.x - 32 * kFEpiWarp0;
    bias_s[et] = a.bias[et];
    asm volatile("bar.sync 1, %0;" ::"n"(32 * kFEpiWarps) : "memory");
    const int q4 = warp & 3, half = (warp - kFEpiWarp0) >> 2;
    const int r = q4 * 32 + lane;
    constexpr float kCorr = (KIND == KBS_KIND_F16) ? (1.0f / kKbsF16LoScale) : 1.0f;
    int j = 0;
    for (int item = blockIdx.x; item < a.items; item += gridDim.x, ++j) {
      const int64_t t = item / ppt, R = int64_t(item % ppt) * kPanelRows + r;
      char* xo = a.x_sb + size_t(t) * a.sbb;
      FTR_WAIT(0, mbar_wait(acc_full, j & 1));
      tc_fence_after();
      const uint32_t tq = tmem_base + (uint32_t(q4 * 32) << 16) + uint32_t(half * 128);
#pragma unroll 1
      for (int cc = 0; cc < 4; ++cc) {
        float v[32], cr[32];
        tmem_ld16(tq + cc * 32, v);
        tmem_ld16(tq + cc * 32 + 16, v + 16);
        tmem_ld16(tq + 256 + cc * 32, cr);
        tmem_ld16(tq + 256 + cc * 32 + 16, cr + 16);
        tmem_ld_wait();
        if (cc == 3) {
          tc_fence_before();
          __syncwarp();
          if (lane == 0) mbar_arrive(acc_empty);
        }
        const float* bs = bias_s + half * 128 + cc * 32;
#pragma unroll
        for (int i = 0; i < 32; ++i) v[i] = (v[i] + kCorr * cr[i]) + bs[i];
        sb_flag_range(a.status, sb_out_of_range<KIND, 32>(v));
#pragma unroll
        for (int c8 = 0; c8 < 4; ++c8) {
          const float x0[4] = {v[8 * c8], v[8 * c8 + 1], v[8 * c8 + 2], v[8 * c8 + 3]};
          const float x1[4] = {v[8 * c8 + 4], v[8 * c8 + 5], v[8 * c8 + 6], v[8 * c8 + 7]};
          if (!(a.dbg & 8))
          sb_store_split8<kPanelRows, KIND>(xo, R, half * 128 + cc * 32 + c8 * 8, a.H / kBlk, sb_split4<KIND>(x0), sb_split4<KIND>(x1),
                                            false);
        }
      }
    }
    if (tr && warp == kFEpiWarp0 && lane == 0) tr[8] = tw[0];
  }
#undef FTR_WAIT
  tc_fence_before();
  __syncthreads();
  if (tr && threadIdx.x == 0) tr[0] = clock64() - t_start;
  if (warp == 0) asm volatile("tcgen05.dealloc.cta_group::1.sync.aligned.b32 %0, %1;" ::"r"(tmem_base), "r"(512u));
}

template <int KIND, int TILE, int GU = 16>
__global__ void __launch_bounds__(256)
pack_lstm_weights_kernel(const float* __restrict__ w_ih, const float* __restrict__ w_hh, const float* __restrict__ b,
                         char* __restrict__ w_sb, float* __restrict__ bias_t, int H, int Kx, int ldx) {
  const int kq = (Kx + H) / 4;
  const int64_t idx = int64_t(blockIdx.x) * 256 + threadIdx.x;
  if (idx >= int64_t(4 * H) * kq) return;
  const int col_g = int(idx / kq);
  const int k = int(idx % kq) * 4;
  const int tile = col_g / TILE, c = col_g % TILE;
  const int grp = c / (4 * GU), gate = (c % (4 * GU)) / GU, uu = c % GU;
  const int u = tile * (TILE / 4) + grp * GU + uu;
  const int row = gate * H + u;
  const float* src = (k < Kx) ? w_ih + size_t(row) * ldx + k : w_hh + size_t(row) * H + (k - Kx);
  const float x[4] = {src[0], src[1], src[2], src[3]};
  sb_store4<TILE, KIND, true>(w_sb, col_g, k, (Kx + H) / kbs_block_k(KIND), x);
  if (k == 0) bias_t[col_g] = b[row];
}

__global__ void __launch_bounds__(256)
fuse_input_weights_kernel(const float* __restrict__ w_ih, const float* __restrict__ w_in, int ld_in, int num_in,
                          const float* __restrict__ b_in, const float* __restrict__ b, float* __restrict__ wf,
                          float* __restrict__ bf, int H, int Kf) {
  const int64_t idx = int64_t(blockIdx.x) * 256 + threadIdx.x;
// ... 1269 lines not shown
  return fn(m, CU_TENSOR_MAP_DATA_TYPE_UINT32, 4, const_cast<char*>(base), gdim, gstride, box, estr, CU_TENSOR_MAP_INTERLEAVE_NONE,
            CU_TENSOR_MAP_SWIZZLE_NONE, CU_TENSOR_MAP_L2_PROMOTION_L2_256B, CU_TENSOR_MAP_FLOAT_OOB_FILL_NONE) == CUDA_SUCCESS;
}

bool kbs_tc_dw_direct_available(const kbs_handle* h, int64_t n) {
  const char* e = getenv("KBS_DW_DIRECT");
  if (e && !atoi(e)) return false;
  return tc_kind(h) == KBS_KIND_F16 && h->p.hidden_size == 256 && (n % kPanelRows) == 0 && tensor_map_encode_fn() != nullptr;
}

int kbs_tc_dw_direct(kbs_handle* h, const KbsTnPlan& plan, const char* dG, const char* x_hist, const char* h_hist, int64_t n, int64_t T,
                     float* partial, float out_scale, cudaStream_t st) {
  const int H = h->p.hidden_size;
  if (!kbs_tc_dw_direct_available(h, n)) return KBS_E_STATE;
  const int panels = int(n / kPanelRows);
  const int64_t units = T * panels;
  if (units > 0x7fffffffLL) return KBS_E_SHAPE;
  if (!h->dw_attr_set) {
    KBS_CUDA_TRY(cudaFuncSetAttribute(dw_gemm_kernel, cudaFuncAttributeMaxDynamicSharedMemorySize, kDwSmemBytes));
    h->dw_attr_set = true;
  }
  DwArgs a{};
  for (int pl = 0; pl < 2; ++pl) {
    if (!encode_sb_plane_map(&a.a_map[pl], dG + pl * (kABlockBytes / 2), 4 * H / 32, units, 4)) return KBS_E_STATE;
    if (!encode_sb_plane_map(&a.b_map[0][pl], x_hist + pl * (kABlockBytes / 2), H / 32, units, 8)) return KBS_E_STATE;
    if (!encode_sb_plane_map(&a.b_map[1][pl], h_hist + pl * (kABlockBytes / 2), H / 32, units, 8)) return KBS_E_STATE;
  }
  a.units = int(units);
  a.ksplit = plan.ksplit;
  a.units_per_run = int((units + plan.ksplit - 1) / plan.ksplit);
  if (int64_t(a.units_per_run) * kPanelRows > 3200 + kPanelRows) return KBS_E_SHAPE;
  a.m_tiles = 4 * H / 128;
  a.partial = partial; a.ldc = 2 * H + 128; a.split_stride = size_t(4 * H) * size_t(a.ldc);
  a.oscale = out_scale;
  const int items = a.m_tiles * 3 * a.ksplit;
  const int grid = items < h->num_sms ? items : h->num_sms;
  KBS_LAUNCH(h, KBS_K_GEMM_TN, st, (dw_gemm_kernel<<<grid, kDwThreads, kDwSmemBytes, st>>>(a)));
  KBS_LAUNCH_CHECK();
  return KBS_OK;
}

int kbs_tc_tn_reduce(kbs_handle* h, const KbsTnPlan& plan, const float* partial, int m_panels, int ldc, int col0, int nrows,
                     int ncols, float* dst, int ld_dst, cudaStream_t st) {
  const int64_t total = int64_t(nrows) * ncols;
  KBS_LAUNCH(h, KBS_K_TN_REDUCE, st, (tn_reduce_kernel<<<unsigned((total + 255) / 256), 256, 0, st>>>(
                                         partial, plan.ksplit, size_t(m_panels) * kPanelRows * size_t(ldc), ldc, col0, nrows, ncols, dst, ld_dst)));
  KBS_LAUNCH_CHECK();
  return KBS_OK;
}

int kbs_tc_tn_reduce_multi(kbs_handle* h, const KbsTnPlan& plan, const float* partial, int m_panels, int ldc, int nrows, int nseg,
                           const int (*seg)[3], float* const* dst, cudaStream_t st) {
  if (nseg < 1 || nseg > 3) return KBS_E_SHAPE;
  TnSegs sg{};
  sg.nseg = nseg;
  for (int k = 0; k < nseg; ++k) {
    sg.col0[k] = seg[k][0]; sg.ncols[k] = seg[k][1]; sg.ld_dst[k] = seg[k][2]; sg.dst[k] = dst[k];
    sg.total_cols += seg[k][1];
  }
  const int64_t total = int64_t(nrows) * sg.total_cols;
  KBS_LAUNCH(h, KBS_K_TN_REDUCE, st, (tn_reduce_multi_kernel<<<unsigned((total + 255) / 256), 256, 0, st>>>(
                                         partial, plan.ksplit, size_t(m_panels) * kPanelRows * size_t(ldc), ldc, nrows, sg)));
  KBS_LAUNCH_CHECK();
  return KBS_OK;
}

size_t kbs_tc_rows_sb_bytes(const kbs_handle* h, int64_t n, int K) { return kbs_sb_bytes_kind(tc_kind(h), pad_rows(n), K); }
int kbs_tc_kind_of(const kbs_handle* h) { return tc_kind(h); }

static size_t rollout_flag_bytes(const kbs_handle* h, int64_t n) {
  return (size_t(h->p.depth + 1) * size_t(pad_rows(n) / kPanelRows) * 4 + 255) / 256 * 256;
}
static size_t rollout_ws_per_net_bytes(const kbs_handle* h, int64_t n) {
  return act_sb_bytes(h, n) * (4 * size_t(h->p.depth)) + 2 * size_t(n) * h->p.hidden_size * 4 +
         2 * size_t(h->p.depth) * size_t(pad_rows(n)) * h->p.hidden_size * 4 + rollout_flag_bytes(h, n) + 256;
}
size_t kbs_tc_rollout_ws_floats(const kbs_handle* h, int64_t n) { return 2 * rollout_ws_per_net_bytes(h, n) / 4; }
int64_t kbs_tc_sb_floats(const kbs_handle* h, int64_t n) { return int64_t(act_sb_bytes(h, n) / 4); }
int64_t kbs_tc_obs_sb_floats(const kbs_handle* h, int net, int64_t n, int64_t T) {
  const int kp = proj_kp(h, net), kf = fused_shape(h, net) ? fused_kp(h, net) : 0;
  return int64_t(kbs_sb_bytes_kind(tc_kind(h), T * pad_rows(n), kp > kf ? kp : kf) / 4);
}

bool kbs_tc_fused_input(const kbs_handle* h, int net, int64_t n, int64_t T, int nets) {
  const char* off_env = getenv("KBS_NO_FUSED_INPUT");
  const char* legacy_env = getenv("KBS_TC_PER_STEP");
  if ((off_env && atoi(off_env)) || (legacy_env && atoi(legacy_env))) return false;
  return fused_shape(h, net) && kbs_tc_persistent_available(h, n, T, nets);
}

int kbs_tc_input_proj_all(kbs_handle* h, int nets, const float* const* obs_soa, float* const* obs_sb, float* const* x_sb_all,
                          int64_t ld, int64_t n, int64_t T, cudaStream_t st, const float* cinert, const float* cvel,
                          KbsTcRolloutArgs* r_out) {
  const int H = h->p.hidden_size, kind = tc_kind(h);
  { const int rc0 = kbs_status_init(h); if (rc0) return rc0; }
  int proj_nets = 0;
  const int64_t np = pad_rows(n);
  static int staged = -1;
  if (staged < 0) { const char* e = getenv("KBS_PROJ_FUSED"); staged = (e && atoi(e)) ? 0 : 1; }
  LayerArgs2 a2{};
  for (int k = 0; k < nets; ++k) {
    const KbsNet& N = h->net[k];
    if (!N.packed || !N.tc_image) return KBS_E_STATE;
    const bool fuse = r_out && kbs_tc_fused_input(h, k, n, T, nets);
    const int Kp = fuse ? fused_kp(h, k) : proj_kp(h, k);
    const float* ci = (k == KBS_NET_CRITIC) ? cinert : nullptr;
    const float* cv = (k == KBS_NET_CRITIC) ? cvel : nullptr;
    char* osb = reinterpret_cast<char*>(obs_sb[k]);
    LayerArgs& a = a2.net[k];
    if (r_out) { r_out->x_sb_all[k] = fuse ? obs_sb[k] : x_sb_all[k]; r_out->x_is_obs[k] = fuse; }
    const char* staged_env = getenv("KBS_PROJ_STAGED");
    if (!fuse && staged && projq_shape(h) && !(staged_env && atoi(staged_env)) && tensor_map_encode_fn()) {
      const int which = (ci && cv && projq_has_dump_layout(h, k)) ? 1 : 0;
      const FLayout Lq = projq_layout(h, k, which);
      FProjArgs fa{};
      const int kf = kbs_block_k(kind);
      bool ok = encode_rows_map(&fa.tmap[0], obs_soa[k], ld, T * int64_t(N.num_in), kf);
      fa.rows_per_step[0] = N.num_in;
      if (which == 1) {
        ok = ok && encode_rows_map(&fa.tmap[1], ci, ld, T * int64_t(10 * KBS_NBODY), kf) &&
             encode_rows_map(&fa.tmap[2], cv, ld, T * int64_t(6 * KBS_NBODY), kf);
        fa.rows_per_step[1] = 10 * KBS_NBODY; fa.rows_per_step[2] = 6 * KBS_NBODY;
      }
      if (ok) {
        fa.kb = Lq.kb; fa.H = H;
        for (int b = 0; b < Lq.kb; ++b) { fa.blk_src[b] = Lq.src[b]; fa.blk_row0[b] = Lq.row0[b]; fa.blk_nvalid[b] = Lq.nvalid[b]; }
        fa.n = n; fa.n_pad = np;
        fa.w_sb = projq_w(h, k, which); fa.bias = projq_bias(h, k, which);
        fa.x_sb = reinterpret_cast<char*>(x_sb_all[k]); fa.sbb = act_sb_bytes(h, n);
        fa.items = int(T * np / kPanelRows);
        fa.status = h->persist_status;
        { const char* e = getenv("KBS_FPROJ_DBG"); fa.dbg = e ? atoi(e) : 0; }
        fa.trace = h->trace_buf;
        const unsigned grid = unsigned(fa.items < h->num_sms ? fa.items : h->num_sms);
        if (kind == KBS_KIND_TF32)
          KBS_LAUNCH(h, KBS_K_PROJ_TC, st, (input_proj_fused_kernel<KBS_KIND_TF32><<<grid, kFThreads, kFSmemBytes, st>>>(fa)));
        else
          KBS_LAUNCH(h, KBS_K_PROJ_TC, st, (input_proj_fused_kernel<KBS_KIND_F16><<<grid, kFThreads, kFSmemBytes, st>>>(fa)));
        continue;
      }
    }
    if (staged || fuse) {
      const int64_t total = T * np * (Kp / 8);
      const unsigned gb = unsigned((total + 255) / 256);
      if (kind == KBS_KIND_TF32)
        KBS_LAUNCH(h, KBS_K_PACK, st, (pack_soa_sb_kernel<KBS_KIND_TF32><<<gb, 256, 0, st>>>(obs_soa[k], N.num_in, ld, osb, n, np, Kp, T, ci, cv, h->persist_status)));
      else
        KBS_LAUNCH(h, KBS_K_PACK, st, (pack_soa_sb_kernel<KBS_KIND_F16><<<gb, 256, 0, st>>>(obs_soa[k], N.num_in, ld, osb, n, np, Kp, T, ci, cv, h->persist_status)));
      a.mode = MODE_PROJ;
      if (fuse) continue;
    } else {
      a.mode = MODE_PROJ_SOA;
      a.soa = obs_soa[k]; a.cinert = ci; a.cvel = cv; a.F = N.num_in; a.soa_ld = ld; a.n_env = n; a.n_pad = np;
    }
    a.x_sb = osb;
    a.h_sb_in = osb;
    a.w_sb = proj_w(h, k);
    a.bias_t = proj_bias(h, k);
    a.x_next_sb = reinterpret_cast<char*>(x_sb_all[k]);
    a.status = h->persist_status;
    a.n = T * np;
    a.H = H; a.kb_x = Kp / kbs_block_k(kind); a.kb_h = 0;
    a.panels = int(T * np / kPanelRows); a.tiles = proj_cols(h) / kTileCols;
    ++proj_nets;
  }
  if (!proj_nets) { KBS_LAUNCH_CHECK(); return KBS_OK; }
  for (int k = 0; k < 2; ++k)
    if (!a2.net[k].panels) a2.net[k].mode = a2.net[k ^ 1].mode;
  KBS_LAUNCH(h, KBS_K_PROJ_TC, st, (launch_layer(h, kind, a2, st)));
  KBS_LAUNCH_CHECK();
  return KBS_OK;
}

bool kbs_tc_persistent_available(const kbs_handle* h, int64_t n, int64_t T, int nets) {
  const int H = h->p.hidden_size, depth = h->p.depth;
  if (!persist_shape_ok(h)) return false;
  const int64_t panels = pad_rows(n) / kPanelRows, tiles = H / kUnitsPerTileP;
  return (T + depth) * int64_t(nets) * panels * (depth * tiles + 1) < (int64_t(1) << 31);
}

int kbs_tc_rollout_recurrent(kbs_handle* h, const KbsTcRolloutArgs& r, cudaStream_t st) {
  const int H = h->p.hidden_size, depth = h->p.depth, kind = tc_kind(h);
  const int nets = r.with_critic ? 2 : 1;
  for (int k = 0; k < nets; ++k)
    if (!h->net[k].packed || !h->net[k].tc_image) return KBS_E_STATE;
  { const int rc0 = kbs_status_init(h); if (rc0) return rc0; }
  const int head_smem = (kHeadEnvs * (H + 4) + KBS_ACTOR_OUT * H + kHeadEnvs * 41 + 4 * 32 * 2) * 4;
  if (!h->head_attr_set) {
    KBS_CUDA_TRY(cudaFuncSetAttribute(rollout_head_kernel, cudaFuncAttributeMaxDynamicSharedMemorySize, 96 * 1024));
    h->head_attr_set = true;
  }
  const int64_t n = r.n, ld = r.ld, np = pad_rows(n);
  const size_t sbb = act_sb_bytes(h, n), per_net = rollout_ws_per_net_bytes(h, n);
  char* hsb[2]; char* xmid[2]; float* h2rm[2]; float* fb[2]; unsigned int* flags[2];
  const size_t fbf = size_t(np) * H;
  for (int k = 0; k < nets; ++k) {
    char* base = reinterpret_cast<char*>(r.ws) + per_net * k;
    hsb[k] = base;
    xmid[k] = base + sbb * 2 * depth;
    h2rm[k] = reinterpret_cast<float*>(xmid[k] + 2 * depth * sbb);
    fb[k] = h2rm[k] + 2 * size_t(n) * H;
    flags[k] = reinterpret_cast<unsigned int*>(fb[k] + 2 * size_t(depth) * fbf);
  }
  const char* legacy_env = getenv("KBS_TC_PER_STEP");
  const int legacy = (legacy_env && !r.save) ? atoi(legacy_env) : 0;
  const bool persistent = !legacy && kbs_tc_persistent_available(h, n, r.T, nets);
  if (r.save) {
    if (!persistent || kind != KBS_KIND_F16 || r.carry_ld) return KBS_E_STATE;
    for (int k = 0; k < nets; ++k) { hsb[k] = r.hsb_hist[k]; xmid[k] = r.xmid_hist[k]; }
  }
  const size_t hstep = r.save ? size_t(r.T + 1) : 2;
  if ((r.x_is_obs[0] || r.x_is_obs[1]) && !persistent) return KBS_E_STATE;
  if (r.mean && !persistent) return KBS_E_STATE;
  if (r.carry_ld && (!persistent || nets * depth * 2 > 8 || H % 8)) return KBS_E_STATE;
  const size_t slot_f = r.carry_ld ? size_t(H) : size_t(n) * H;
  if (nets * depth * 2 <= 8 && H % 8 == 0) {
    CarryJobs J{};
    J.ld_rm = r.carry_ld ? r.carry_ld : H;
    J.status = h->persist_status;
    int j = 0;
    for (int k = 0; k < nets; ++k)
      for (int l = 0; l < depth; ++l) {
        char* h_dst = hsb[k] + sbb * (hstep * l);
        float* c_dst = r.save ? r.c_hist[k] + fbf * (hstep * l) : fb[k] + fbf * (2 * l);
        if (!r.carry[k]) {
          KBS_CUDA_TRY(cudaMemsetAsync(h_dst, 0, sbb, st));
          KBS_CUDA_TRY(cudaMemsetAsync(c_dst, 0, fbf * sizeof(float), st));
          continue;
        }
        J.rm[j] = r.carry[k] + (size_t(l) * 2 + 0) * slot_f; J.blk[j] = h_dst; J.mode[j++] = 0;
        J.rm[j] = r.carry[k] + (size_t(l) * 2 + 1) * slot_f; J.blk[j] = c_dst; J.mode[j++] = 1;
      }
    if (j) carry_convert(h, J, j, n, np, H, st);
  } else {
    for (int k = 0; k < nets; ++k)
      for (int l = 0; l < depth; ++l) {
        pack_rows(h, r.carry[k] + (size_t(l) * 2 + 0) * size_t(n) * H, H, hsb[k] + sbb * (2 * l), n, np, H, st);
        fb_convert(h, r.carry[k] + (size_t(l) * 2 + 1) * size_t(n) * H, fb[k] + fbf * (2 * l), n, np, H, 1, st);
      }
  }
  const int panels = int(np / kPanelRows), tiles = H / kUnitsPerTileP;
  if (persistent) {
    if (r.chunk_len > 0)
      for (int64_t c = 0; c * r.chunk_len < r.T; ++c) KBS_CUDA_TRY(cudaStreamWaitEvent(st, r.chunk_events[c], 0));
    PArgs a{};
    for (int k = 0; k < nets; ++k) {
      PNet& N = a.net[k];
      N.x_sb_all = reinterpret_cast<const char*>(r.x_sb_all[k]);
      N.kb_x0 = r.x_is_obs[k] ? fused_kp(h, k) / kbs_block_k(kind) : H / kbs_block_k(kind);
      N.x0_stride = r.x_is_obs[k] ? kbs_sb_bytes_kind(kind, np, fused_kp(h, k)) : sbb;
      N.hsb = hsb[k]; N.xmid = xmid[k]; N.fb = fb[k]; N.flags = flags[k];
      N.c_hist = r.save ? r.c_hist[k] : nullptr; N.save_g = r.save ? r.save_g[k] : nullptr;
      for (int l = 0; l < depth; ++l) { N.w_sb[l] = layer_w_p(h, k, l); N.bias_t[l] = layer_bias_p(h, k, l); }
      if (r.x_is_obs[k]) { N.w_sb[0] = fused_w(h, k); N.bias_t[0] = fused_bias(h, k); }
      N.w_head = head_w(h, k); N.bias_head = head_bias(h, k);
      KBS_CUDA_TRY(cudaMemsetAsync(flags[k], 0, rollout_flag_bytes(h, n), st));
    }
    a.nets = nets; a.depth = depth; a.H = H; a.panels = panels; a.tiles = tiles;
    a.n = n; a.ld = ld; a.T = r.T; a.sbb = sbb;
    {
      int gp = panels;
      const char* e = getenv("KBS_PERSIST_GROUP");
      if (e) { const int v = atoi(e); gp = (v <= 0 || v > panels) ? panels : v; }
      a.gpanels = gp;
    }
    a.done = r.done;
    a.arm_cmd = r.actor_obs + size_t(55) * ld;
    a.lpf = r.lpf; a.eps = r.eps_action;
    a.q = r.qpos ? r.qpos + size_t(7) * ld : nullptr;
    a.qd = r.qvel ? r.qvel + size_t(6) * ld : nullptr;
    a.ep = r.ep;
    a.action = r.action; a.log_prob = r.log_prob; a.ctrl = (r.ctrl && r.qpos && r.qvel) ? r.ctrl : nullptr; a.value = r.value;
    a.action_in = r.action_in; a.entropy = r.entropy; a.std = r.action_std; a.mean = r.mean;
    a.sraw = r.save ? r.sraw : nullptr; a.hist = r.save ? 1 : 0;
    a.status = h->persist_status;
    { const char* e = getenv("KBS_PERSIST_DBG"); a.dbg = e ? atoi(e) : 0; }
    a.trace = h->trace_buf;
    cudaLaunchConfig_t cfg{};
    const int64_t per_slot = int64_t(nets) * a.gpanels * (depth * tiles + 1);
    cfg.gridDim = dim3(unsigned(per_slot < h->num_sms ? per_slot : h->num_sms));
    { const char* e = getenv("KBS_PERSIST_GRID"); if (e && atoi(e) > 0 && atoi(e) < int(cfg.gridDim.x)) cfg.gridDim.x = unsigned(atoi(e)); }
    cfg.blockDim = dim3(kThreadsP);
    cfg.dynamicSmemBytes = kPSmemBytes;
    cfg.stream = st;
    cudaLaunchAttribute at[1];
    at[0].id = cudaLaunchAttributeCooperative;
    at[0].val.cooperative = 1;
    cfg.attrs = at;
    cfg.numAttrs = 1;
    cudaError_t le = cudaSuccess;
    if (r.save)
      KBS_LAUNCH(h, KBS_K_ROLLOUT_TC, st, (le = cudaLaunchKernelEx(&cfg, rollout_persist_kernel<KBS_KIND_F16, true>, h->p, a)));
    else if (kind == KBS_KIND_TF32)
      KBS_LAUNCH(h, KBS_K_ROLLOUT_TC, st, (le = cudaLaunchKernelEx(&cfg, rollout_persist_kernel<KBS_KIND_TF32, false>, h->p, a)));
    else
      KBS_LAUNCH(h, KBS_K_ROLLOUT_TC, st, (le = cudaLaunchKernelEx(&cfg, rollout_persist_kernel<KBS_KIND_F16, false>, h->p, a)));
    KBS_CUDA_TRY(le);
    { const int rc0 = kbs_status_publish(h, st); if (rc0) return rc0; }
    if (r.save) { KBS_LAUNCH_CHECK(); return KBS_OK; }
    if (nets * depth * 2 <= 8 && H % 8 == 0) {
      CarryJobs J{};
      J.ld_rm = r.carry_ld ? r.carry_ld : H;
      J.status = nullptr;
      int j = 0;
      for (int k = 0; k < nets; ++k) {
        float* dst = (r.carry_ld && r.carry_out[k]) ? r.carry_out[k] : r.carry[k];
        for (int l = 0; l < depth; ++l) {
          J.rm[j] = dst + (size_t(l) * 2 + 1) * slot_f; J.blk[j] = fb[k] + fbf * (2 * l); J.mode[j++] = 2;
          J.rm[j] = dst + (size_t(l) * 2 + 0) * slot_f; J.blk[j] = fb[k] + fbf * (2 * l + 1); J.mode[j++] = 2;
        }
      }
      carry_convert(h, J, j, n, np, H, st);
    } else {
      for (int k = 0; k < nets; ++k)
        for (int l = 0; l < depth; ++l) {
          fb_convert(h, r.carry[k] + (size_t(l) * 2 + 1) * size_t(n) * H, fb[k] + fbf * (2 * l), n, np, H, 0, st);
          fb_convert(h, r.carry[k] + (size_t(l) * 2 + 0) * size_t(n) * H, fb[k] + fbf * (2 * l + 1), n, np, H, 0, st);
        }
    }
    KBS_LAUNCH_CHECK();
    return KBS_OK;
  }
  { const int rc0 = kbs_side_stream_init(h); if (rc0) return rc0; }
  cudaStream_t side = h->side_stream;
  for (int64_t t = 0; t < r.T; ++t) {
    const int pin = int(t & 1), pout = pin ^ 1;
    const uint8_t* done_t = r.done ? r.done + t * ld : nullptr;
    if (r.chunk_len > 0 && t % r.chunk_len == 0) KBS_CUDA_TRY(cudaStreamWaitEvent(st, r.chunk_events[t / r.chunk_len], 0));
    if (t >= 2) KBS_CUDA_TRY(cudaStreamWaitEvent(st, h->ev_head[pin], 0));
    for (int l = 0; l < depth; ++l) {
      LayerArgs2 a2{};
      for (int k = 0; k < nets; ++k) {
        LayerArgs& a = a2.net[k];
        fill_lstm_args(h, k, l, a);
        a.x_sb = (l == 0) ? reinterpret_cast<const char*>(r.x_sb_all[k]) + size_t(t) * sbb : xmid[k] + sbb * ((l - 1) & 1);
        a.h_sb_in = hsb[k] + sbb * (2 * l + pin);
        a.h_sb_out = hsb[k] + sbb * (2 * l + pout);
        a.c = fb[k] + fbf * (2 * l);
        a.h_carry = fb[k] + fbf * (2 * l + 1);
        a.x_next_sb = (l + 1 < depth) ? xmid[k] + sbb * (l & 1) : nullptr;
        a.h_next_rm = (l + 1 < depth) ? nullptr : h2rm[k] + size_t(pin) * n * H;
        a.done = done_t;
        a.n = n;
        a.panels = int(np / kPanelRows);
        if (h->trace_buf && t == h->trace_step && l == h->trace_layer) a.trace = h->trace_buf;
      }
      KBS_LAUNCH(h, KBS_K_LSTM_TC, st, (launch_layer(h, kind, a2, st)));
    }
    KBS_CUDA_TRY(cudaEventRecord(h->ev_lstm[pin], st));
    KBS_CUDA_TRY(cudaStreamWaitEvent(side, h->ev_lstm[pin], 0));
    HeadArgs ha{};
    for (int k = 0; k < nets; ++k) {
      ha.h2[k] = h2rm[k] + size_t(pin) * n * H; ha.w_out[k] = h->net[k].w_out; ha.b_out[k] = h->net[k].b_out;
    }
    ha.arm_cmd = r.actor_obs + (size_t(t) * KBS_ACTOR_OBS + 55) * ld;
    ha.lpf = r.lpf;
    ha.eps = r.eps_action ? r.eps_action + size_t(t) * KBS_NUM_JOINTS * ld : nullptr;
    ha.done = done_t;
    ha.q = r.qpos ? r.qpos + (size_t(t) * KBS_NQ + 7) * ld : nullptr;
    ha.qd = r.qvel ? r.qvel + (size_t(t) * KBS_NV + 6) * ld : nullptr;
    ha.ep = r.ep;
    ha.action = r.action ? r.action + size_t(t) * KBS_NUM_JOINTS * ld : nullptr;
    ha.log_prob = r.log_prob ? r.log_prob + size_t(t) * ld : nullptr;
    ha.ctrl = r.ctrl ? r.ctrl + size_t(t) * KBS_NUM_JOINTS * ld : nullptr;
    ha.value = r.value ? r.value + size_t(t) * ld : nullptr;
    ha.action_in = r.action_in ? r.action_in + size_t(t) * KBS_NUM_JOINTS * ld : nullptr;
    ha.entropy = r.entropy ? r.entropy + size_t(t) * ld : nullptr;
    ha.std = r.action_std ? r.action_std + size_t(t) * KBS_NUM_JOINTS * ld : nullptr;
    ha.n = n; ha.ld = ld; ha.H = H;
    static int skip_head = -1;
    if (skip_head < 0) { const char* e = getenv("KBS_SKIP_HEAD"); skip_head = e ? atoi(e) : 0; }
    if (!skip_head)
    KBS_LAUNCH(h, KBS_K_ACTOR_HEAD, side,
               (rollout_head_kernel<<<dim3(unsigned((n + kHeadEnvs - 1) / kHeadEnvs), unsigned(nets)), 128, head_smem, side>>>(
                   h->p, ha)));
    KBS_CUDA_TRY(cudaEventRecord(h->ev_head[pin], side));
  }
  KBS_CUDA_TRY(cudaStreamWaitEvent(st, h->ev_head[0], 0));
  if (r.T > 1) KBS_CUDA_TRY(cudaStreamWaitEvent(st, h->ev_head[1], 0));
  for (int k = 0; k < nets; ++k)
    for (int l = 0; l < depth; ++l) {
      fb_convert(h, r.carry[k] + (size_t(l) * 2 + 1) * size_t(n) * H, fb[k] + fbf * (2 * l), n, np, H, 0, st);
      fb_convert(h, r.carry[k] + (size_t(l) * 2 + 0) * size_t(n) * H, fb[k] + fbf * (2 * l + 1), n, np, H, 0, st);
    }
  KBS_LAUNCH_CHECK();
  return KBS_OK;
}

int kbs_tc_debug_trace(kbs_handle* h, long long* trace_out, float* ws, int64_t n, cudaStream_t st) {
  const int H = h->p.hidden_size;
  for (int k = 0; k < 2; ++k)
    if (!h->net[k].packed || !h->net[k].tc_image) return KBS_E_STATE;
  const int64_t np = pad_rows(n);
  const size_t sbb = act_sb_bytes(h, n);
  char* wsb = reinterpret_cast<char*>(ws);
  KBS_CUDA_TRY(cudaMemsetAsync(wsb, 0, sbb * 4 + size_t(np) * H * 4 * 3, st));
  float* rm = reinterpret_cast<float*>(wsb + sbb * 4);
  LayerArgs2 a2{};
  for (int k = 0; k < 2; ++k) {
    LayerArgs& a = a2.net[k];
    fill_lstm_args(h, k, 0, a);
    a.x_sb = wsb; a.h_sb_in = wsb + sbb; a.h_sb_out = wsb + 2 * sbb; a.x_next_sb = wsb + 3 * sbb;
    a.c = rm; a.h_carry = rm + size_t(np) * H; a.h_next_rm = nullptr; a.done = nullptr; a.n = n;
    a.trace = trace_out;
    a.panels = int(np / kPanelRows);
  }
  KBS_LAUNCH(h, KBS_K_LSTM_TC, st, (launch_layer(h, tc_kind(h), a2, st)));
  KBS_LAUNCH_CHECK();
  return KBS_OK;
}
```

### kbot-joystick_b200/csrc/kbs_ppo_update.cu

```cuda
#include <math.h>

#include "kbs_common.cuh"

namespace {

constexpr int kT = 256;
inline int round_up_i(int x, int m) { return (x + m - 1) / m * m; }

__global__ void __launch_bounds__(kT)
soa_to_rows_kernel(const float* __restrict__ soa, int F, int64_t ld, float* __restrict__ rm, int kp, int64_t n, int64_t T) {
  const int64_t idx = int64_t(blockIdx.x) * kT + threadIdx.x;
  if (idx >= T * n * kp) return;
  const int f = int(idx % kp);
  const int64_t row = idx / kp;
  const int64_t t = row / n, e = row - t * n;
  rm[idx] = f < F ? soa[(t * F + f) * ld + e] : 0.0f;
}

__global__ void __launch_bounds__(kT)
transpose_kernel(const float* __restrict__ in, int rows, int cols, float* __restrict__ out) {
  const int64_t idx = int64_t(blockIdx.x) * kT + threadIdx.x;
  if (idx >= int64_t(rows) * cols) return;
  const int r = int(idx / cols), c = int(idx % cols);
  out[size_t(c) * rows + r] = in[idx];
// ... 871 lines not shown
  { const int rc0 = kbs_side_stream_init(h); if (rc0) return rc0; }
  int side_pack = 1;
  { const char* e = getenv("KBS_PPO_SIDE_PACK"); if (e) side_pack = atoi(e); }
  cudaStream_t ss = side_pack ? h->side_stream : st;
  if (side_pack) {
    KBS_CUDA_TRY(cudaEventRecord(h->ev_pre, st));
    KBS_CUDA_TRY(cudaStreamWaitEvent(ss, h->ev_pre, 0));
  }
  float gscale = 16.0f;
  while (gscale < 16.0f * float(rows)) gscale *= 2.0f;
  const bool rank1_critic = narrow && h->net[1].num_out == 1;
  for (int k = 1; k >= 0; --k) {
    const KbsNet& N = h->net[k];
    const int kpp = round_up_i(N.num_in + 1, 128);
    if ((rc = kbs_tc_soa_to_tn(h, plan, k == 0 ? b.actor_obs : b.critic_obs, N.num_in, ld, n, T, kpp, true, w[k].tnb_obs, ss))) return rc;
    if (!(k == 1 && rank1_critic))
      KBS_LAUNCH(h, KBS_K_PACK, ss, (transpose_kernel<<<blocks(int64_t(64) * H), kT, 0, ss>>>(N.w_out, 64, H, w[k].w_outT)));
    if ((rc = kbs_tc_pack_bwd(h, k, ss, kbs_tc_bptt_tile(h, n)))) return rc;
    KBS_CUDA_TRY(cudaMemsetAsync(w[k].dc, 0, size_t(depth) * npH * 4, ss));
    KBS_CUDA_TRY(cudaMemsetAsync(w[k].bflags, 0, kbs_tc_bptt_flag_bytes(h, n), ss));
    for (int l = 0; l < depth; ++l)
      KBS_CUDA_TRY(cudaMemsetAsync(w[k].dG + (size_t(l) * (T + 1) + T) * sb4, 0, sb4, ss));
    if (kb_used < plan.kb_total)
      for (int l = 0; l < depth; ++l)
        for (int c = 0; c < 4 * H / 128; ++c)
          KBS_CUDA_TRY(cudaMemsetAsync(w[k].tna_dG[l] + size_t(c) * plan.col_bytes + size_t(kb_used) * 16384, 0,
                                       size_t(plan.kb_total - kb_used) * 16384, ss));
    KBS_CUDA_TRY(cudaMemsetAsync(w[k].tn_zero, 0, 1024 * sizeof(float), ss));
    if ((rc = kbs_tc_ones_block(h, w[k].tn_ones, ss))) return rc;
  }
  if (side_pack) KBS_CUDA_TRY(cudaEventRecord(h->ev_lstm[0], ss));
  {
    const float* obs_soa[2] = {b.actor_obs, b.critic_obs};
    float* xsb[2] = {reinterpret_cast<float*>(w[0].x_sb), reinterpret_cast<float*>(w[1].x_sb)};
    if ((rc = kbs_tc_input_proj_all(h, 2, obs_soa, osb, xsb, ld, n, T, st, nullptr, nullptr, nullptr))) return rc;
  }
  if (narrow) {
    KbsFwdSaveArgs fa{};
    for (int k = 0; k < 2; ++k) {
      KbsFwdSaveNet& F = fa.net[k];
      F.x0 = w[k].x_sb; F.xmid = w[k].xmid; F.hsb = w[k].hsb; F.c_hist = w[k].c_hist; F.save_g = w[k].save_g;
      F.h_top_rm = w[k].h_top_rm; F.flags = w[k].fflags; F.carry0 = k == 0 ? b.actor_carry0 : b.critic_carry0;
      for (int l = 0; l < depth; ++l) F.tn_xh[l] = w[k].tnb_layer[l];
      if (kb_used < plan.kb_total)
        for (int l = 0; l < depth; ++l)
          for (int c = 0; c < 2 * H / 128; ++c)
            KBS_CUDA_TRY(cudaMemsetAsync(w[k].tnb_layer[l] + size_t(c) * plan.col_bytes + size_t(kb_used) * 16384, 0,
                                         size_t(plan.kb_total - kb_used) * 16384, st));
    }
    fa.nets = 2; fa.n = n; fa.ld = ld; fa.T = T; fa.done = b.done; fa.tn_plan = dw_direct ? nullptr : &plan;
    fa.transposed_out = &xh_transposed;
    if ((rc = kbs_tc_fwd_save(h, fa, st))) return rc;
    if ((rc = kbs_simt_gemm_nt(h, w[0].h_top_rm, H, h->net[0].w_out, H, h->net[0].b_out, w[0].out, 64, rows, 64, H, 0, st))) return rc;
    {
      const size_t head_smem = size_t(T) * 32 * 4 * 3 + size_t(T) + 16;
      static int block_head = -1;
      if (block_head < 0) { const char* e = getenv("KBS_PPO_HEAD_BLOCK"); block_head = e ? atoi(e) : 1; }
      if (block_head && head_smem <= 48 * 1024)
        KBS_LAUNCH(h, KBS_K_ACTOR_HEAD, st,
                   (actor_head_fwd_bwd_block_kernel<<<unsigned(n), 128, head_smem, st>>>(
                       h->p, L, w[0].out, b.actor_obs, b.action, b.done, b.lpf0, b.old_log_probs, b.advantages, y_s, sd_s, log_probs,
                       entropy, w[0].dout, T, ld, n)));
      else
        KBS_LAUNCH(h, KBS_K_ACTOR_HEAD, st,
                   (actor_head_fwd_bwd_warp_kernel<<<unsigned((n + 3) / 4), 128, 0, st>>>(
                       h->p, L, w[0].out, b.actor_obs, b.action, b.done, b.lpf0, b.old_log_probs, b.advantages, y_s, sd_s, log_probs,
                       entropy, w[0].dout, T, ld, n)));
    }
    if (rank1_critic) {
      KBS_LAUNCH(h, KBS_K_CRITIC_HEAD, st,
                 (critic_value_head_kernel<<<unsigned((rows + 7) / 8), 256, 0, st>>>(L, w[1].h_top_rm, h->net[1].w_out, h->net[1].b_out,
                                                                                    b.old_values, b.value_targets, values, w[1].dout,
                                                                                    w[1].out , H, T, ld, n)));
    } else {
      if ((rc = kbs_simt_gemm_nt(h, w[1].h_top_rm, H, h->net[1].w_out, H, h->net[1].b_out, w[1].out, 64, rows, 64, H, 0, st))) return rc;
      KBS_LAUNCH(h, KBS_K_CRITIC_HEAD, st,
                 (critic_head_fwd_bwd_kernel<<<blocks(rows), kT, 0, st>>>(L, w[1].out, b.old_values, b.value_targets, values, w[1].dout, T, ld, n)));
    }
  } else {
    KbsTcRolloutArgs r{};
    r.x_sb_all[0] = reinterpret_cast<float*>(w[0].x_sb); r.x_sb_all[1] = reinterpret_cast<float*>(w[1].x_sb);
    r.n = n; r.ld = ld; r.T = T; r.with_critic = true;
    r.carry[0] = const_cast<float*>(b.actor_carry0); r.carry[1] = const_cast<float*>(b.critic_carry0);
    r.done = b.done; r.actor_obs = b.actor_obs;
    if (b.lpf0) KBS_CUDA_TRY(cudaMemcpyAsync(lpf, b.lpf0, size_t(KBS_NUM_JOINTS) * ld * 4, cudaMemcpyDeviceToDevice, st));
    else KBS_CUDA_TRY(cudaMemsetAsync(lpf, 0, size_t(KBS_NUM_JOINTS) * ld * 4, st));
    r.lpf = lpf;
    r.action_in = b.action; r.log_prob = log_probs; r.entropy = entropy; r.action_std = sd_s; r.mean = y_s; r.value = values;
    r.ws = ws;
    r.save = 1; r.sraw = sraw_s;
    for (int k = 0; k < 2; ++k) { r.xmid_hist[k] = w[k].xmid; r.hsb_hist[k] = w[k].hsb; r.c_hist[k] = w[k].c_hist; r.save_g[k] = w[k].save_g; }
    if ((rc = kbs_tc_rollout_recurrent(h, r, st))) return rc;
    KBS_LAUNCH(h, KBS_K_ACTOR_HEAD, st,
               (actor_head_bwd_warp_kernel<<<unsigned((n + 3) / 4), 128, 0, st>>>(h->p, L, b.action, b.done, b.old_log_probs, b.advantages,
                                                                                 y_s, sd_s, sraw_s, log_probs, w[0].dout, T, ld, n)));
    KBS_LAUNCH(h, KBS_K_CRITIC_HEAD, st,
               (critic_head_bwd_kernel<<<blocks(rows), kT, 0, st>>>(L, values, b.old_values, b.value_targets, w[1].dout, T, ld, n)));
  }
  if (side_pack) {
    KBS_CUDA_TRY(cudaEventRecord(h->ev_lstm[1], st));
    KBS_CUDA_TRY(cudaStreamWaitEvent(ss, h->ev_lstm[1], 0));
  }
  for (int k = 1; k >= 0; --k) {
    for (int l = 0; l < depth && !xh_transposed && !dw_direct; ++l) {
      const char* x_hist = l == 0 ? w[k].x_sb : w[k].xmid + size_t(l - 1) * T * sbb;
      if ((rc = kbs_tc_sb_to_tn(h, plan, true, x_hist, sbb, kbH, 0, kbH, n, T, w[k].tnb_layer[l], ss))) return rc;
      if ((rc = kbs_tc_sb_to_tn(h, plan, true, w[k].hsb + size_t(l) * (T + 1) * sbb, sbb, kbH, 0, kbH, n, T,
                                w[k].tnb_layer[l] + size_t(H / 128) * plan.col_bytes, ss)))
        return rc;
    }
    if (narrow) {
      if ((rc = kbs_tc_pack_tn(h, plan, true, w[k].h_top_rm, H, 0, H, H, rows, w[k].tnb_top, 1.0f, -1, ss, n, np))) return rc;
    } else if ((rc = kbs_tc_sb_to_tn(h, plan, true, w[k].xmid + size_t(depth - 1) * T * sbb, sbb, kbH, 0, kbH, n, T, w[k].tnb_top, ss))) {
      return rc;
    }
    if ((rc = kbs_tc_pack_tn(h, plan, false, w[k].dout, 64, 0, 64, 128, rows, w[k].tn_a, gscale, -1, ss, n, np))) return rc;
  }
  if (side_pack) KBS_CUDA_TRY(cudaEventRecord(h->ev_head[0], ss));
  if (side_pack) KBS_CUDA_TRY(cudaStreamWaitEvent(st, h->ev_lstm[0], 0));
  KbsBpttArgs ba{};
  for (int k = 0; k < 2; ++k) {
    KbsBpttNet& B = ba.net[k];
    if (k == 1 && rank1_critic) {
      B.dh_top = nullptr; B.dv = w[1].out; B.w_out = h->net[1].w_out;
    } else {
      if ((rc = kbs_simt_gemm_nt(h, w[k].dout, 64, w[k].w_outT, 64, nullptr, w[k].dh_top, H, rows, H, 64, 0, st))) return rc;
      B.dh_top = w[k].dh_top;
    }
    B.dG = w[k].dG; B.save_g = w[k].save_g; B.c_hist = w[k].c_hist; B.dx = w[k].dx; B.dx0 = w[k].dx0;
    B.dc = w[k].dc; B.flags = w[k].bflags;
    for (int l = 0; l < depth; ++l) B.tn_dG[l] = w[k].tna_dG[l];
  }
  ba.nets = 2; ba.n = n; ba.ld = ld; ba.T = T; ba.done = b.done; ba.gscale = gscale;
  bool dG_transposed = false;
  ba.tn_plan = dw_direct ? nullptr : &plan; ba.transposed_out = &dG_transposed;
  if ((rc = kbs_tc_bptt(h, ba, st))) return rc;
  if (side_pack) KBS_CUDA_TRY(cudaStreamWaitEvent(st, h->ev_head[0], 0));
  const float inv = 1.0f / gscale;
  if (side_pack) {
    KBS_CUDA_TRY(cudaEventRecord(h->ev_head[1], st));
    KBS_CUDA_TRY(cudaStreamWaitEvent(ss, h->ev_head[1], 0));
  }
  for (int k = 1; k >= 0; --k) {
    const KbsNet& N = h->net[k];
    const kbs_net_grads* g = grads[k];
    cudaStream_t sk = k == 1 ? ss : st;
    for (int l = 0; l < depth; ++l) {
      const int mp = 4 * H / 128, ldc = (2 * H / 128 + 1) * 128;
      if (dw_direct) {
        const char* x_hist = l == 0 ? w[k].x_sb : w[k].xmid + size_t(l - 1) * T * sbb;
        if ((rc = kbs_tc_dw_direct(h, plan, w[k].dG + size_t(l) * (T + 1) * sb4, x_hist, w[k].hsb + size_t(l) * (T + 1) * sbb, n, T,
                                   w[k].tn_partial, inv, sk)))
          return rc;
      } else {
        if (!dG_transposed &&
            (rc = kbs_tc_sb_to_tn(h, plan, false, w[k].dG + size_t(l) * (T + 1) * sb4, sb4, kb4, 0, kb4, n, T, w[k].tna_dG[l], sk)))
          return rc;
        if ((rc = kbs_tc_gemm_tn(h, plan, w[k].tna_dG[l], mp, 4 * H, w[k].tnb_layer[l], 2 * H / 128, w[k].tn_ones, w[k].tn_zero,
                                 w[k].tn_partial, inv, sk)))
          return rc;
      }
      {
        const int sg3[3][3] = {{0, H, H}, {H, H, H}, {2 * H, 1, 1}};
        float* const dst3[3] = {g->w_ih[l], g->w_hh[l], g->b[l]};
        if ((rc = kbs_tc_tn_reduce_multi(h, plan, w[k].tn_partial, mp, ldc, 4 * H, 3, sg3, dst3, sk))) return rc;
      }
    }
// ... 194 lines not shown
```

Before: 69.53 million.

## Write actor observations directly into split-operand layout and skip half-empty weight blocks

The observation kernel now emits actor observations straight into the tensor-core operand panel layout (split hi/lo), using per-warp shared-memory transposes. This removes the separate SoA actor-obs buffer and its repack pass in the input projection. The arm command read by the recurrent kernel now comes from the command tensor through a configurable stride, since actor_obs may no longer exist. The fused input GEMM also loads only half of each weight block and skips the second half of the UMMA issues when a K block has at most half its features valid. The cost is a more complex obs kernel with shared memory and warp syncs.

```diff
diff --git a/kbot-joystick_b200/csrc/kbs_api.cu b/kbot-joystick_b200/csrc/kbs_api.cu
--- a/kbot-joystick_b200/csrc/kbs_api.cu
+++ b/kbot-joystick_b200/csrc/kbs_api.cu
@@ -92,10 +92,11 @@
     if (chunks_cfg < 1 || chunks_cfg > kKbsMaxChunks) chunks_cfg = 1;
   }
   const int64_t CT = (T + chunks_cfg - 1) / chunks_cfg;
+  const bool actor_direct = chunks_cfg == 1 && kbs_tc_fused_input(h, KBS_NET_ACTOR, n, T, critic ? 2 : 1);
   const size_t sbf = size_t(kbs_tc_sb_floats(h, n));
   const size_t ws_f = kbs_tc_rollout_ws_floats(h, n);
   const size_t lag_f = io->pg_carry ? size_t(T) * 3 * ld : 0;
-  const size_t aobs_f = io->actor_obs ? 0 : size_t(T) * KBS_ACTOR_OBS * ld;
+  const size_t aobs_f = (io->actor_obs || actor_direct) ? 0 : size_t(T) * KBS_ACTOR_OBS * ld;
   const size_t cobs_f = critic ? size_t(CT) * KBS_CRITIC_OBS * ld : 0;
   const size_t xsb_f = size_t(T) * sbf;
   const size_t osb_a_f = size_t(kbs_tc_obs_sb_floats(h, KBS_NET_ACTOR, n, CT));
@@ -104,7 +105,7 @@
   if (rc) return rc;
   float* ws = h->scratch;
   float* lagged = io->pg_carry ? ws + ws_f : nullptr;
-  float* aobs = io->actor_obs ? io->actor_obs : ws + ws_f + lag_f;
+  float* aobs = io->actor_obs ? io->actor_obs : (actor_direct ? nullptr : ws + ws_f + lag_f);
   float* cobs = critic ? ws + ws_f + lag_f + aobs_f : nullptr;
   float* xsb_a = ws + ws_f + lag_f + aobs_f + cobs_f;
   float* xsb_c = critic ? xsb_a + xsb_f : nullptr;
@@ -134,12 +135,13 @@
     const int64_t tc = (T - t0 < CT) ? T - t0 : CT;
     const kbs_state_view s = state_at(io->state, t0);
     const kbs_noise_view nz = noise_at(io->noise, t0, ld);
-    float* aobs_c = aobs + t0 * KBS_ACTOR_OBS * ld;
+    float* aobs_c = aobs ? aobs + t0 * KBS_ACTOR_OBS * ld : nullptr;
     if ((rc = kbs_launch_observations(h, s, &nz, &io->episode, io->command + t0 * KBS_NUM_COMMANDS * ld, nullptr, nullptr,
                                       nullptr, aobs_c, cobs, n, aux, tc, lagged ? lagged + t0 * 3 * ld : nullptr,
-                                      true)))
+                                      true, actor_direct ? osb_a : nullptr,
+                                      kbs_tc_fused_kp(h, KBS_NET_ACTOR))))
       return rc;
-    const float* obs_soa[2] = {aobs_c, cobs};
+    const float* obs_soa[2] = {actor_direct ? nullptr : aobs_c, cobs};
     float* obs_sb[2] = {osb_a, osb_c};
     float* xsb[2] = {xsb_a + size_t(t0) * sbf, critic ? xsb_c + size_t(t0) * sbf : nullptr};
     if ((rc = kbs_tc_input_proj_all(h, critic ? 2 : 1, obs_soa, obs_sb, xsb, ld, n, tc, aux,
@@ -151,7 +153,8 @@
   r.chunk_len = overlap ? CT : 0; r.chunk_events = h->ev_chunk;
   r.n = n; r.ld = ld; r.T = T; r.with_critic = critic;
   r.carry[0] = io->actor_carry; r.carry[1] = io->critic_carry;
-  r.done = io->done; r.actor_obs = aobs; r.lpf = io->lpf; r.eps_action = io->eps_action;
+  r.done = io->done; r.lpf = io->lpf; r.eps_action = io->eps_action;
+  r.arm_cmd = io->command + 6 * ld; r.arm_cmd_step = KBS_NUM_COMMANDS * ld;
   r.qpos = io->state.qpos; r.qvel = io->state.qvel; r.ep = io->episode;
   r.action = io->action; r.log_prob = io->log_prob; r.ctrl = io->ctrl; r.value = io->value;
   r.ws = ws;
@@ -655,7 +658,7 @@
       if ((rc = kbs_tc_input_proj_all(h, 1, obs_soa, obs_sb, x_all, ld, n, 1, st, nullptr, nullptr, &r))) return rc;
       r.n = n; r.ld = ld; r.T = 1; r.with_critic = false;
       r.carry[0] = const_cast<float*>(carry_in); r.carry_out[0] = carry_out; r.carry_ld = carry_w;
-      r.actor_obs = obs; r.lpf = lpf; r.action = act;
+      r.arm_cmd = obs + 55 * ld; r.arm_cmd_step = KBS_ACTOR_OBS * ld; r.lpf = lpf; r.action = act;
       r.ws = ws;
       if ((rc = kbs_tc_rollout_recurrent(h, r, st))) return rc;
       return kbs_launch_policy_unpack(h, nullptr, lpf, act, carry_out, action_out, ld, n, st);
@@ -731,7 +734,8 @@
   }
   r.n = n; r.ld = ld; r.T = T; r.with_critic = critic;
   r.carry[0] = io->actor_carry; r.carry[1] = io->critic_carry;
-  r.done = io->done; r.actor_obs = io->actor_obs; r.lpf = io->lpf;
+  r.done = io->done; r.lpf = io->lpf;
+  r.arm_cmd = io->actor_obs + 55 * ld; r.arm_cmd_step = KBS_ACTOR_OBS * ld;
   r.action_in = io->action; r.log_prob = io->log_probs; r.entropy = io->entropy; r.action_std = io->action_std;
   r.mean = io->mean;
   r.value = io->values;
diff --git a/kbot-joystick_b200/csrc/kbs_common.cuh b/kbot-joystick_b200/csrc/kbs_common.cuh
--- a/kbot-joystick_b200/csrc/kbs_common.cuh
+++ b/kbot-joystick_b200/csrc/kbs_common.cuh
@@ -102,7 +102,8 @@
 int kbs_launch_observations(kbs_handle* h, const kbs_state_view& s, const kbs_noise_view* nz,
                             const kbs_episode_view* ep, const float* command, float* pg_carry,
                             const uint8_t* pg_reset, float* computed, float* actor_obs, float* critic_obs, int64_t n,
-                            cudaStream_t st, int64_t T = 1, const float* pg_lagged = nullptr, bool skip_dump = false);
+                            cudaStream_t st, int64_t T = 1, const float* pg_lagged = nullptr, bool skip_dump = false,
+                            float* actor_sb = nullptr, int actor_sb_kp = 0);
 int kbs_launch_ppo_loss(kbs_handle* h, const kbs_ppo_loss_params& L, const kbs_ppo_loss_io& io, int64_t n, cudaStream_t st);
 int kbs_launch_ppo_loss_at(kbs_handle* h, const kbs_ppo_loss_params& L, const kbs_ppo_loss_io& io, int64_t n, double* partials,
                            cudaStream_t st);
@@ -171,7 +172,8 @@
   int64_t carry_ld;
   float* carry_out[2];
   const uint8_t* done;
-  const float* actor_obs;
+  const float* arm_cmd;
+  int64_t arm_cmd_step;
   float* lpf;
   const float* eps_action;
   const float* qpos;
@@ -195,6 +197,7 @@
                           int64_t ld, int64_t n, int64_t T, cudaStream_t st, const float* cinert = nullptr,
                           const float* cvel = nullptr, struct KbsTcRolloutArgs* r_out = nullptr);
 bool kbs_tc_fused_input(const kbs_handle* h, int net, int64_t n, int64_t T, int nets);
+int kbs_tc_fused_kp(const kbs_handle* h, int net);
 int kbs_tc_rollout_recurrent(kbs_handle* h, const KbsTcRolloutArgs& r, cudaStream_t st);
 bool kbs_tc_persistent_available(const kbs_handle* h, int64_t n, int64_t T, int nets);
 int kbs_tc_debug_trace(kbs_handle* h, long long* trace_out, float* ws, int64_t n, cudaStream_t st);
diff --git a/kbot-joystick_b200/csrc/kbs_elementwise.cu b/kbot-joystick_b200/csrc/kbs_elementwise.cu
--- a/kbot-joystick_b200/csrc/kbs_elementwise.cu
+++ b/kbot-joystick_b200/csrc/kbs_elementwise.cu
@@ -60,17 +60,54 @@
 
 constexpr int kCopyRowsPerSection = 46;
 constexpr int kObsSections = 4;
+constexpr int kObsSbSmem = kThreads / 32 * 8 * 32 * 16;
+static_assert(kThreads % 32 == 0 && 32 * 4 == kKbsPanelRows, "obs_kernel: one warp's envs are one operand panel");
+
+struct ObsSb {
+  char* sb;
+  int kind, kblocks;
+  int64_t n_pad;
+  unsigned int* status;
+};
+
+template <int KIND>
+__device__ __forceinline__ void obs_sb_chunk_k(const ObsSb& o, float4 (*tile)[32], const float (&v)[8][4], int c, bool zero,
+                                               int64_t t, int64_t n0, int64_t n, unsigned mask, int nlive) {
+  const int lane = threadIdx.x & 31;
+  const int64_t p0 = n0 - 4 * lane;
+  if (!zero) {
+#pragma unroll
+    for (int i = 0; i < 8; ++i) tile[i][lane] = make_float4(v[i][0], v[i][1], v[i][2], v[i][3]);
+  }
+  __syncwarp(mask);
+  for (int r = lane; r < kKbsPanelRows; r += nlive) {
+    float x[8];
+#pragma unroll
+    for (int i = 0; i < 8; ++i) x[i] = (!zero && p0 + r < n) ? reinterpret_cast<const float*>(tile[i])[r] : 0.0f;
+    sb_flag_range(o.status, sb_out_of_range<KIND, 8>(x));
+    const float x0[4] = {x[0], x[1], x[2], x[3]}, x1[4] = {x[4], x[5], x[6], x[7]};
+    sb_store_split8<kKbsPanelRows, KIND>(o.sb, t * o.n_pad + p0 + r, c * 8, o.kblocks, sb_split4<KIND>(x0), sb_split4<KIND>(x1),
+                                         zero);
+  }
+  __syncwarp(mask);
+}
+__device__ __forceinline__ void obs_sb_chunk(const ObsSb& o, float4 (*tile)[32], const float (&v)[8][4], int c, bool zero,
+                                             int64_t t, int64_t n0, int64_t n, unsigned mask, int nlive) {
+  if (o.kind == KBS_KIND_F16) obs_sb_chunk_k<KBS_KIND_F16>(o, tile, v, c, zero, t, n0, n, mask, nlive);
+  else obs_sb_chunk_k<KBS_KIND_TF32>(o, tile, v, c, zero, t, n0, n, mask, nlive);
+}
 
 __global__ void __launch_bounds__(kThreads)
 obs_kernel(const __grid_constant__ kbs_params P, kbs_state_view s, kbs_noise_view nz,
            const kbs_episode_view ep, const float* __restrict__ command, float* __restrict__ pg_carry,
            const uint8_t* __restrict__ pg_reset, const float* __restrict__ pg_lagged, float* __restrict__ computed,
-           float* __restrict__ actor_obs, float* __restrict__ critic_obs, int64_t n) {
+           float* __restrict__ actor_obs, float* __restrict__ critic_obs, int64_t n, const ObsSb osb) {
+  extern __shared__ float4 sb_tiles[];
   const int64_t n0 = (int64_t(blockIdx.x) * kThreads + threadIdx.x) * 4;
   if (n0 >= n) return;
   const int64_t ld = s.ld;
+  const int64_t t = blockIdx.z;
   {
-    const int64_t t = blockIdx.z;
     s.qpos += t * KBS_NQ * ld; s.qvel += t * KBS_NV * ld; s.sensordata += t * KBS_NSENSORDATA * ld;
     s.xpos += t * 3 * KBS_NBODY * ld; s.xquat += t * 4 * KBS_NBODY * ld;
     if (s.cinert) s.cinert += t * 10 * KBS_NBODY * ld;
@@ -96,31 +133,60 @@
   }
 
   const bool has_noise = nz.eps_jpos != nullptr;
-
-  if (sec < 2) {
-#pragma unroll 5
-  for (int j = sec * 10; j < sec * 10 + 10; ++j) {
-    float q[4], qd[4], jb[4] = {0, 0, 0, 0}, e1[4] = {0, 0, 0, 0}, e2[4] = {0, 0, 0, 0};
-    kbs_ld4(s.qpos, 7 + j, ld, n0, q);
-    kbs_ld4(s.qvel, 6 + j, ld, n0, qd);
-    if (ep.jpos_bias) kbs_ld4(ep.jpos_bias, j, ld, n0, jb);
-    if (has_noise) { kbs_ld4(nz.eps_jpos, j, ld, n0, e1); kbs_ld4(nz.eps_jvel, j, ld, n0, e2); }
-    float bj[4], nbj[4], nv[4], a0[4], a1[4], c0[4], c1[4];
-#pragma unroll
-    for (int l = 0; l < 4; ++l) {
-      bj[l] = q[l] + jb[l];
-      nbj[l] = bj[l] + P.jpos_noise_mag * e1[l];
-      nv[l] = qd[l] + P.jvel_noise_mag * e2[l];
-      a0[l] = (nbj[l] - P.joint_bias[j]) / P.joint_range[j];
-      a1[l] = nv[l] / 10.0f;
-      c0[l] = (q[l] - P.joint_bias[j]) / P.joint_range[j];
-      c1[l] = qd[l] / 10.0f;
-    }
-    if (computed) { kbs_st4(computed, j, ld, n0, bj); kbs_st4(computed, 20 + j, ld, n0, nbj); kbs_st4(computed, 40 + j, ld, n0, nv); }
-    if (actor_obs) { kbs_st4(actor_obs, j, ld, n0, a0); kbs_st4(actor_obs, 20 + j, ld, n0, a1); }
-    if (critic_obs) { kbs_st4(critic_obs, j, ld, n0, c0); kbs_st4(critic_obs, 20 + j, ld, n0, c1); }
-  }
-  return;
+  float4 (*tile)[32] = reinterpret_cast<float4 (*)[32]>(sb_tiles + (threadIdx.x >> 5) * 8 * 32);
+  const int64_t p0 = n0 - 4 * (threadIdx.x & 31);
+  const int nlive = n - p0 >= 128 ? 32 : int((n - p0 + 3) / 4);
+  const unsigned live_mask = nlive == 32 ? 0xffffffffu : (1u << nlive) - 1u;
+
+  if (sec < 3) {
+    const int c_end = sec < 2 ? 2 * sec + 2 : 5;
+    for (int c = 2 * sec; c < c_end; ++c) {
+      float av[8][4];
+#pragma unroll
+      for (int i = 0; i < 8; ++i) {
+        const int f = 8 * c + i;
+        if (f < 20) {
+          const int j = f;
+          float q[4], jb[4] = {0, 0, 0, 0}, e1[4] = {0, 0, 0, 0}, bj[4], nbj[4], c0[4];
+          kbs_ld4(s.qpos, 7 + j, ld, n0, q);
+          if (ep.jpos_bias) kbs_ld4(ep.jpos_bias, j, ld, n0, jb);
+          if (has_noise) kbs_ld4(nz.eps_jpos, j, ld, n0, e1);
+#pragma unroll
+          for (int l = 0; l < 4; ++l) {
+            bj[l] = q[l] + jb[l];
+            nbj[l] = bj[l] + P.jpos_noise_mag * e1[l];
+            av[i][l] = (nbj[l] - P.joint_bias[j]) / P.joint_range[j];
+            c0[l] = (q[l] - P.joint_bias[j]) / P.joint_range[j];
+          }
+          if (computed) { kbs_st4(computed, j, ld, n0, bj); kbs_st4(computed, 20 + j, ld, n0, nbj); }
+          if (actor_obs) kbs_st4(actor_obs, j, ld, n0, av[i]);
+          if (critic_obs) kbs_st4(critic_obs, j, ld, n0, c0);
+        } else {
+          const int j = f - 20;
+          float qd[4], e2[4] = {0, 0, 0, 0}, nv[4], c1[4];
+          kbs_ld4(s.qvel, 6 + j, ld, n0, qd);
+          if (has_noise) kbs_ld4(nz.eps_jvel, j, ld, n0, e2);
+#pragma unroll
+          for (int l = 0; l < 4; ++l) {
+            nv[l] = qd[l] + P.jvel_noise_mag * e2[l];
+            av[i][l] = nv[l] / 10.0f;
+            c1[l] = qd[l] / 10.0f;
+          }
+          if (computed) kbs_st4(computed, 40 + j, ld, n0, nv);
+          if (actor_obs) kbs_st4(actor_obs, 20 + j, ld, n0, av[i]);
+          if (critic_obs) kbs_st4(critic_obs, 20 + j, ld, n0, c1);
+        }
+      }
+      if (osb.sb) obs_sb_chunk(osb, tile, av, c, false, t, n0, n, live_mask, nlive);
+    }
+  }
+  if (sec == 0) {
+    if (osb.sb) {
+      const float none[8][4] = {};
+      const int c_end = osb.kblocks * (osb.kind == KBS_KIND_F16 ? 32 : 16) / 8;
+      for (int c = 9; c < c_end; ++c) obs_sb_chunk(osb, tile, none, c, true, t, n0, n, live_mask, nlive);
+    }
+    return;
   }
 
   if (sec == 2) {
@@ -185,9 +251,21 @@
       for (int k = 0; k < 5; ++k) kbs_st4(critic_obs, 40 + k, ld, n0, enc_c[k]);
       for (int k = 0; k < 3; ++k) kbs_st4(critic_obs, 45 + k, ld, n0, gy[k]);
     }
-  }
-
-  if (sec == 2) {
+    if (osb.sb) {
+      float av[8][4];
+#pragma unroll
+      for (int l = 0; l < 4; ++l) {
+#pragma unroll
+        for (int k = 0; k < 5; ++k) av[k][l] = enc_a[k][l];
+#pragma unroll
+        for (int k = 0; k < 3; ++k) av[5 + k][l] = o_ngy[k][l];
+      }
+      obs_sb_chunk(osb, tile, av, 5, false, t, n0, n, live_mask, nlive);
+    }
+    return;
+  }
+
+  if (sec == 1) {
   float c[16][4];
 #pragma unroll
   for (int k = 0; k < 16; ++k) kbs_ld4(command, k, ld, n0, c[k]);
@@ -203,6 +281,29 @@
     kbs_st4(critic_obs, 48, ld, n0, zc);
 #pragma unroll
     for (int k = 0; k < 16; ++k) kbs_st4(critic_obs, 49 + k, ld, n0, c[k]);
+  }
+  if (osb.sb) {
+    float av[8][4];
+#pragma unroll
+    for (int l = 0; l < 4; ++l) {
+      av[0][l] = zc[l];
+#pragma unroll
+      for (int k = 0; k < 7; ++k) av[1 + k][l] = c[k][l];
+    }
+    obs_sb_chunk(osb, tile, av, 6, false, t, n0, n, live_mask, nlive);
+#pragma unroll
+    for (int l = 0; l < 4; ++l) {
+#pragma unroll
+      for (int k = 0; k < 8; ++k) av[k][l] = c[7 + k][l];
+    }
+    obs_sb_chunk(osb, tile, av, 7, false, t, n0, n, live_mask, nlive);
+#pragma unroll
+    for (int l = 0; l < 4; ++l) {
+      av[0][l] = c[15][l];
+#pragma unroll
+      for (int k = 1; k < 8; ++k) av[k][l] = 0.0f;
+    }
+    obs_sb_chunk(osb, tile, av, 8, false, t, n0, n, live_mask, nlive);
   }
   return;
   }
@@ -1281,14 +1382,25 @@
 int kbs_launch_observations(kbs_handle* h, const kbs_state_view& s, const kbs_noise_view* nz,
                             const kbs_episode_view* ep, const float* command, float* pg_carry,
                             const uint8_t* pg_reset, float* computed, float* actor_obs, float* critic_obs, int64_t n,
-                            cudaStream_t st, int64_t T, const float* pg_lagged, bool skip_dump) {
+                            cudaStream_t st, int64_t T, const float* pg_lagged, bool skip_dump, float* actor_sb,
+                            int actor_sb_kp) {
   kbs_noise_view z{};
   kbs_episode_view e{};
   if (nz) z = *nz;
   if (ep) e = *ep;
+  ObsSb o{};
+  if (actor_sb) {
+    const int rc = kbs_status_init(h);
+    if (rc) return rc;
+    o.sb = reinterpret_cast<char*>(actor_sb);
+    o.kind = kbs_tc_kind_of(h);
+    o.kblocks = actor_sb_kp / kbs_block_k(o.kind);
+    o.n_pad = (n + kKbsPanelRows - 1) / kKbsPanelRows * kKbsPanelRows;
+    o.status = h->persist_status;
+  }
   dim3 grid(groups4(n), (critic_obs && !skip_dump) ? kObsSections + 368 / kCopyRowsPerSection : kObsSections, unsigned(T));
-  KBS_LAUNCH(h, KBS_K_OBS, st, (obs_kernel<<<grid, kThreads, 0, st>>>(h->p, s, z, e, command, pg_carry, pg_reset, pg_lagged,
-                                                                      computed, actor_obs, critic_obs, n)));
+  KBS_LAUNCH(h, KBS_K_OBS, st, (obs_kernel<<<grid, kThreads, o.sb ? kObsSbSmem : 0, st>>>(h->p, s, z, e, command, pg_carry,
+                                                                      pg_reset, pg_lagged, computed, actor_obs, critic_obs, n, o)));
   KBS_LAUNCH_CHECK();
   return KBS_OK;
 }
diff --git a/kbot-joystick_b200/csrc/kbs_net_tc.cu b/kbot-joystick_b200/csrc/kbs_net_tc.cu
--- a/kbot-joystick_b200/csrc/kbs_net_tc.cu
+++ b/kbot-joystick_b200/csrc/kbs_net_tc.cu
@@ -658,6 +658,7 @@
   size_t sbb;
   const uint8_t* done;
   const float* arm_cmd;
+  int64_t arm_cmd_step;
   float* lpf;
   const float* eps;
   const float* q; const float* qd;
@@ -1080,7 +1081,7 @@
               const int64_t o = jn * ld + e;
               in_lpf[jj] = __ldcg(args.lpf + o);
               in_eps[jj] = args.eps ? __ldg(args.eps + t * KBS_NUM_JOINTS * ld + o) : 0.0f;
-              in_arm[jj] = (jn >= 10) ? __ldg(args.arm_cmd + t * KBS_ACTOR_OBS * ld + (jn - 10) * ld + e) : 0.0f;
+              in_arm[jj] = (jn >= 10) ? __ldg(args.arm_cmd + t * args.arm_cmd_step + (jn - 10) * ld + e) : 0.0f;
               in_ain[jj] = args.action_in ? __ldg(args.action_in + t * KBS_NUM_JOINTS * ld + o) : 0.0f;
               if (args.ctrl) {
                 in_q[jj] = __ldg(args.q + t * KBS_NQ * ld + o);
@@ -2030,9 +2031,9 @@
         for (int b = 0; b < a.kb; ++b, ++g) {
           const int s = g % kFStagesOp;
           FTR_WAIT(0, mbar_wait(&empty[s], ((g / kFStagesOp) & 1) ^ 1));
-          mbar_expect_tx(&full[s], uint32_t(kFOpBytes - kABlockBytes));
-          bulk_g2s(op + size_t(s) * kFOpBytes + kABlockBytes, a.w_sb + size_t(b) * (kFOpBytes - kABlockBytes),
-                   uint32_t(kFOpBytes - kABlockBytes), &full[s]);
+          const uint32_t wb = uint32_t(kFOpBytes - kABlockBytes) / (a.blk_nvalid[b] > kFeat / 2 ? 1 : 2);
+          mbar_expect_tx(&full[s], wb);
+          bulk_g2s(op + size_t(s) * kFOpBytes + kABlockBytes, a.w_sb + size_t(b) * (kFOpBytes - kABlockBytes), wb, &full[s]);
         }
       }
       if (tr) tr[3] = tw[0];
@@ -2101,15 +2102,18 @@
         const uint64_t a_hi = umma_desc(sa, 2048, 128), a_lo = a_hi + (8192 >> 4);
         const uint64_t b_hi = umma_desc(sa + kABlockBytes, 8192, 128), b_lo = b_hi + (4096 >> 4);
         constexpr uint64_t kAStep = 4096 >> 4, kBStep = 16384 >> 4;
+        const bool second = a.blk_nvalid[b] > kFeat / 2;
         if (elect_one()) {
           const uint32_t acc = b != 0;
           if (!(a.dbg & 2)) {
           umma<KIND, 256>(d_main, a_hi, b_hi, acc);
           umma<KIND, 256>(d_corr, a_lo, b_hi, acc);
           umma<KIND, 256>(d_corr, a_hi, b_lo, 1);
+          if (second) {
           umma<KIND, 256>(d_main, a_hi + kAStep, b_hi + kBStep, 1);
           umma<KIND, 256>(d_corr, a_lo + kAStep, b_hi + kBStep, 1);
           umma<KIND, 256>(d_corr, a_hi + kAStep, b_lo + kBStep, 1);
+          }
           }
           umma_commit(&empty[s]);
         }
@@ -3545,6 +3549,7 @@
   return int64_t(kbs_sb_bytes_kind(tc_kind(h), T * pad_rows(n), kp > kf ? kp : kf) / 4);
 }
 
+int kbs_tc_fused_kp(const kbs_handle* h, int net) { return fused_kp(h, net); }
 bool kbs_tc_fused_input(const kbs_handle* h, int net, int64_t n, int64_t T, int nets) {
   const char* off_env = getenv("KBS_NO_FUSED_INPUT");
   const char* legacy_env = getenv("KBS_TC_PER_STEP");
@@ -3572,6 +3577,10 @@
     char* osb = reinterpret_cast<char*>(obs_sb[k]);
     LayerArgs& a = a2.net[k];
     if (r_out) { r_out->x_sb_all[k] = fuse ? obs_sb[k] : x_sb_all[k]; r_out->x_is_obs[k] = fuse; }
+    if (!obs_soa[k]) {
+      if (!fuse) return KBS_E_STATE;
+      continue;
+    }
     const char* staged_env = getenv("KBS_PROJ_STAGED");
     if (!fuse && staged && projq_shape(h) && !(staged_env && atoi(staged_env)) && tensor_map_encode_fn()) {
       const int which = (ci && cv && projq_has_dump_layout(h, k)) ? 1 : 0;
@@ -3728,7 +3737,7 @@
       a.gpanels = gp;
     }
     a.done = r.done;
-    a.arm_cmd = r.actor_obs + size_t(55) * ld;
+    a.arm_cmd = r.arm_cmd; a.arm_cmd_step = r.arm_cmd_step;
     a.lpf = r.lpf; a.eps = r.eps_action;
     a.q = r.qpos ? r.qpos + size_t(7) * ld : nullptr;
     a.qd = r.qvel ? r.qvel + size_t(6) * ld : nullptr;
@@ -3816,7 +3825,7 @@
     for (int k = 0; k < nets; ++k) {
       ha.h2[k] = h2rm[k] + size_t(pin) * n * H; ha.w_out[k] = h->net[k].w_out; ha.b_out[k] = h->net[k].b_out;
     }
-    ha.arm_cmd = r.actor_obs + (size_t(t) * KBS_ACTOR_OBS + 55) * ld;
+    ha.arm_cmd = r.arm_cmd + size_t(t) * r.arm_cmd_step;
     ha.lpf = r.lpf;
     ha.eps = r.eps_action ? r.eps_action + size_t(t) * KBS_NUM_JOINTS * ld : nullptr;
     ha.done = done_t;
diff --git a/kbot-joystick_b200/csrc/kbs_ppo_update.cu b/kbot-joystick_b200/csrc/kbs_ppo_update.cu
--- a/kbot-joystick_b200/csrc/kbs_ppo_update.cu
+++ b/kbot-joystick_b200/csrc/kbs_ppo_update.cu
@@ -977,7 +977,7 @@
     r.x_sb_all[0] = reinterpret_cast<float*>(w[0].x_sb); r.x_sb_all[1] = reinterpret_cast<float*>(w[1].x_sb);
     r.n = n; r.ld = ld; r.T = T; r.with_critic = true;
     r.carry[0] = const_cast<float*>(b.actor_carry0); r.carry[1] = const_cast<float*>(b.critic_carry0);
-    r.done = b.done; r.actor_obs = b.actor_obs;
+    r.done = b.done; r.arm_cmd = b.actor_obs + 55 * ld; r.arm_cmd_step = KBS_ACTOR_OBS * ld;
     if (b.lpf0) KBS_CUDA_TRY(cudaMemcpyAsync(lpf, b.lpf0, size_t(KBS_NUM_JOINTS) * ld * 4, cudaMemcpyDeviceToDevice, st));
     else KBS_CUDA_TRY(cudaMemsetAsync(lpf, 0, size_t(KBS_NUM_JOINTS) * ld * 4, st));
     r.lpf = lpf;
```

After: 69.56 million, median of 6. Within noise of the previous version (+0.0%).
